# ratt-ru/tricolour

Hardware: AMD Instinct MI355X
Metric: Mvis/s flagged (bl x time x chan x corr) (higher is better)
Workload: dtype f32 data / f64 accumulators / u8 flags; 1 GPU; MeerKAT-64 slab: 252 of 2016 bl x 4 corr x 1024 time x 4096 chan per GPU (BASELINE configs[1] processed as HBM-resident baseline slabs), sum_threshold_flagger kwargs=stage1; params=stage1

## Files before the change

tricolour_amd/csrc/kernels_boxline.hpp:

```cpp
#pragma once

struct BoxDenom { float b, y; };
__device__ __forceinline__ float box_divide(float a, const BoxDenom dn, unsigned long long& okmask) {
    float q = a * dn.y;
    okmask &= __builtin_amdgcn_ballot_w64(__builtin_amdgcn_classf(q, 0x148));
    float r = __builtin_fmaf(-dn.b, q, a);
    q = __builtin_fmaf(r, dn.y, q);
    r = __builtin_fmaf(-dn.b, q, a);
    q = __builtin_fmaf(r, dn.y, q);
    return q;
}
__device__ __forceinline__ float box_divide_ieee(float a, const BoxDenom dn) { return a / dn.b; }
__device__ __forceinline__ float box_divide_checked(float a, const BoxDenom dn) {
    unsigned long long ok = ~0ull;
    const float q = box_divide(a, dn, ok);
    return ((ok >> (threadIdx.x & 63)) & 1ull) ? q : box_divide_ieee(a, dn);
}

template <int KS, typename V, typename A>
struct BoxLine {
    V R1[KS], R2[KS], R3[KS], R4[KS];
    A s1, s2, s3, s4;
    V o1, o2, o3;
    V old1, old2, old3, old4;
// ... 116 lines not shown
                const unsigned w = (unsigned)__builtin_amdgcn_raw_buffer_load_b32(frs, coff, t < n ? (int)((unsigned)(t >> 2) * rowb) : 0, 0);
                prew[q] = (t < n) ? w : 0x01010101u;
            }
        } else {
#pragma unroll
            for (int u = 0; u < PF; u++) {
                const int t = t0 + u;
                const unsigned w = (unsigned)__builtin_amdgcn_raw_buffer_load_b8(frs, c, t < n ? (int)((unsigned)t * (unsigned)C) : 0, 0);
                prew[PACKED ? 0 : u] = (t < n) ? w : 1u;
            }
        }
        if (IMG == 1) {
#pragma unroll
            for (int u = 0; u < PF; u++)
                pre[u] = __builtin_bit_cast(float, __builtin_amdgcn_raw_buffer_load_b32(drs, coff, t0 + u < n ? (int)((unsigned)(t0 + u) * rowb) : 0, 0));
        }
    };
    auto store = [&](int i, float y) {
        __builtin_amdgcn_raw_buffer_store_b32(__builtin_bit_cast(unsigned, y), ors, coff, (int)((unsigned)i * rowb), 0);
    };
    issue(0);
    for (int mb = 0; mb < total; mb += UNR) {
#pragma unroll
        for (int b = 0; b < UNR / PF; b++) {
            const int m0 = mb + b * PF;
            if (m0 < total) {
                V cur[PF];
#pragma unroll
                for (int u = 0; u < PF; u++) {
                    const bool fl = PACKED ? ((prew[u >> 2] >> (8 * (u & 3))) & 0xFFu) != 0 : prew[PACKED ? 0 : u] != 0;
                    cur[u] = (IMG == 0) ? (fl ? (V)0 : (V)1) : (fl ? (V)0 : (V)pre[u]);
                }
                issue(m0 + PF);
                const bool fast = SPLIT && m0 >= 4 * r + 3 && m0 + PF <= n;
                if (fast) {
#pragma unroll
                    for (int u = 0; u < PF; u++) {
                        V* cell = cells + (size_t)lslot * BT4;
                        if (HASL) lslot = (lslot + 1 == d) ? 0 : lslot + 1;
                        const V* ncell = cells + (size_t)lslot * BT4;
                        const float out = boxline_step<KS, V, A, HASL, true>(L, (b * PF + u) % KS, m0 + u, cur[u], n, R2x, cell, ncell, BT);
                        store(m0 + u - 3 - 4 * r, out / denom);
                        if (BOXR_SCHED_EVERY > 0 && (u % (BOXR_SCHED_EVERY > 0 ? BOXR_SCHED_EVERY : 1)) == (BOXR_SCHED_EVERY > 0 ? BOXR_SCHED_EVERY : 1) - 1) __builtin_amdgcn_sched_barrier(0);
                    }
                } else {
#pragma unroll
                    for (int u = 0; u < PF; u++) {
                        V* cell = cells + (size_t)lslot * BT4;
                        if (HASL) lslot = (lslot + 1 == d) ? 0 : lslot + 1;
                        const V* ncell = cells + (size_t)lslot * BT4;
                        const float out = boxline_step<KS, V, A, HASL, false>(L, (b * PF + u) % KS, m0 + u, cur[u], n, R2x, cell, ncell, BT);
                        const int i = m0 + u - 3 - 4 * r;
                        if (i >= 0 && i < n) store(i, out / denom);
                        if (BOXR_SCHED_EVERY > 0 && (u % (BOXR_SCHED_EVERY > 0 ? BOXR_SCHED_EVERY : 1)) == (BOXR_SCHED_EVERY > 0 ? BOXR_SCHED_EVERY : 1) - 1) __builtin_amdgcn_sched_barrier(0);
                    }
                }
            }
        }
    }
}

template <int KS, bool HASL, int IMG>
__global__ void __launch_bounds__(64, boxr_waves(KS))
k_boxt(const float* __restrict__ srcData, const uint8_t* __restrict__ srcFlags,
       float* __restrict__ dstImg, int n, int C, int r, float denom, size_t sws, size_t dws) {
    boxt_body<KS, HASL, IMG, true, boxr_pf(KS)>(srcData, srcFlags, dstImg, n, C, r, denom, sws, dws, blockIdx.y);
}

__host__ __device__ constexpr int boxt_spec_pf(int ks) { return ks <= 16 ? 64 : (ks == 32 ? 32 : 16); }
template <int KS, bool HASL>
__global__ void __launch_bounds__(64, 1)
k_boxt_spec(const float* __restrict__ srcData, const uint8_t* __restrict__ srcFlags,
            float* __restrict__ dstW, float* __restrict__ dstO, int n, int C, int r, float denom) {
    if (blockIdx.y == 0) boxt_body<KS, HASL, 0, false, boxt_spec_pf(KS)>(srcData, srcFlags, dstW, n, C, r, denom, 0, 0, 0);
    else boxt_body<KS, HASL, 1, false, boxt_spec_pf(KS)>(srcData, srcFlags, dstO, n, C, r, denom, 0, 0, 0);
}

__host__ __device__ constexpr int boxf_ts(int pf) { return pf >= 32 ? 33 : 34; }
#ifndef BOXF_DOUBLE_STAGE
#define BOXF_DOUBLE_STAGE 1
#endif
__host__ __device__ constexpr int boxf_nsub(int ks) { return (BOXF_DOUBLE_STAGE && ks <= 16 && boxr_pf_f(ks) == 16) ? 2 : 1; }
#define BOXF_TS 34
#ifndef BOXF_STREAM_AUX
#define BOXF_STREAM_AUX 0
#endif
__host__ __device__ constexpr bool boxf_panel_ok(int ks, bool hasl) { return ks <= 8 || (ks == 16 && !hasl); }
template <int KS, bool HASL, int MODE, int WPS = boxr_waves_f(KS)>
__global__ void __launch_bounds__(64, WPS)
k_boxf(const float* __restrict__ srcW, unsigned img_gap,
       float* __restrict__ dstW, float* __restrict__ dstO, const float* __restrict__ data,
       int n, int C, int ld, int r, BoxDenom denom, size_t sws_img, size_t dws, size_t ws_data,
       uint8_t* __restrict__ nanflag, float* __restrict__ dstP, size_t pws) {
    extern __shared__ float cf_ring[];
    constexpr int PF = boxr_pf_f(KS);
    static_assert(MODE != 2 || (PF / 2) % 4 == 0, "panel output: groups of four positions per lane");
    constexpr int NSUB = boxf_nsub(KS);
    constexpr int PL = PF * NSUB;
    constexpr int UNR = boxr_lcm(boxr_lcm(KS, PF), PL);
    constexpr int BT = 64;
    constexpr int LPI = 32 / PL;
    constexpr int TS = boxf_ts(PL);
    const int lane = threadIdx.x;
    const int half = lane >> 5;
    const int hl = lane & 31;
    const int c0 = blockIdx.x * 32;
    const int c = c0 + hl;
    const bool colok = c < C;
    const size_t win = blockIdx.y;
    const int R2x = 2 * r;
    const int d = R2x - KS;
    float* ring = cf_ring + lane;
    float* tiles = cf_ring + (size_t)4 * d * BT;
    float* tile = tiles + (size_t)half * PL * TS;
    if (HASL)
        for (int k = 0; k < 4 * d; k++) ring[(size_t)k * BT] = 0.0f;

    const unsigned rowb = (unsigned)C * 4u;
    const __amdgpu_buffer_rsrc_t xrs = __builtin_amdgcn_make_buffer_rsrc(
        (void*)(data + win * ws_data), 0, (int)((unsigned)n * rowb), 0x00020000);
    const __amdgpu_buffer_rsrc_t ors = __builtin_amdgcn_make_buffer_rsrc(
        (void*)(dstO + win * dws), 0, (int)((unsigned)n * rowb), 0x00020000);
    const __amdgpu_buffer_rsrc_t wrs = __builtin_amdgcn_make_buffer_rsrc(
        (void*)(dstW + win * dws), 0, (int)((unsigned)n * rowb), 0x00020000);
    const bool panel = MODE == 2 && boxf_panel_ok(KS, HASL) && dstP != nullptr;
    const __amdgpu_buffer_rsrc_t prs = __builtin_amdgcn_make_buffer_rsrc(
        (void*)(panel ? dstP + win * pws : dstW), 0, panel ? (int)((unsigned)n * rowb) : 0, 0x00020000);

    const int s_pos = hl % PL;
    const int s_line0 = hl / PL;
    const unsigned ldb = (unsigned)ld * 4u;
    const __amdgpu_buffer_rsrc_t srs = __builtin_amdgcn_make_buffer_rsrc(
        (void*)(srcW + win * sws_img), 0, (int)((img_gap + (unsigned)C * (unsigned)ld) * 4u), 0x00020000);
    const int s_off = (int)((unsigned)s_line0 * ldb) + s_pos * 4 + (half ? (int)(img_gap * 4u) : 0);
    float pre[PL];
    auto issue = [&](int t0) {
        const int sbase = (int)((unsigned)c0 * ldb) + t0 * 4;
        if (t0 + PL <= n && c0 + 32 <= C) {
#pragma unroll
            for (int j = 0; j < PL; j++)
                pre[j] = __builtin_bit_cast(float, __builtin_amdgcn_raw_buffer_load_b32(srs, s_off, sbase + (int)((unsigned)(LPI * j) * ldb), 0));
        } else {
            const bool tok = t0 + s_pos < n;
#pragma unroll
            for (int j = 0; j < PL; j++) {
                const bool ok = tok && (c0 + LPI * j + s_line0 < C);
                const float v = __builtin_bit_cast(float, __builtin_amdgcn_raw_buffer_load_b32(srs, ok ? s_off + sbase + (int)((unsigned)(LPI * j) * ldb) : 0, 0, 0));
                pre[j] = ok ? v : 0.0f;
            }
        }
    };
    auto wave_sync = [] {
        __builtin_amdgcn_fence(__ATOMIC_RELEASE, "wavefront");
        __builtin_amdgcn_wave_barrier();
        __builtin_amdgcn_fence(__ATOMIC_ACQUIRE, "wavefront");
    };
    const int hrow = (PF / 2) * half;
    const int hoff = (colok ? c : 0) * 4 + (int)((unsigned)hrow * rowb);
    const float* eb = tiles + (size_t)hrow * TS + hl;
    float dpre[PF / 2];
    auto issue_data = [&](int m0, bool fast) {
        const int i0 = m0 - 3 - 4 * r;
        if (fast) {
#pragma unroll
            for (int k = 0; k < PF / 2; k++)
                dpre[k] = __builtin_bit_cast(float, __builtin_amdgcn_raw_buffer_load_b32(xrs, hoff, (int)((unsigned)(i0 + k) * rowb), BOXF_STREAM_AUX));
        } else {
#pragma unroll
            for (int k = 0; k < PF / 2; k++) {
                const int i = i0 + hrow + k;
                const bool ok = i >= 0 && i < n;
                const float v = __builtin_bit_cast(float, __builtin_amdgcn_raw_buffer_load_b32(xrs, ok ? (colok ? c : 0) * 4 + (int)((unsigned)i * rowb) : 0, 0, 0));
                dpre[k] = ok ? v : 0.0f;
            }
        }
    };

    BoxLine<KS, float, double> L;
    L.init();
    constexpr size_t BT4 = (size_t)4 * BT;
    int lslot = 0;
    const int total = n + 4 * r + 3;
    bool line_nan = false;
    issue(0);
    for (int mb = 0; mb < total; mb += UNR) {
#pragma unroll
        for (int b = 0; b < UNR / PF; b++) {
            const int m0 = mb + b * PF;
            if (m0 < total) {
                const int ro = (b % NSUB) * PF;
                if (b % NSUB == 0) {
                    wave_sync();
#pragma unroll
                    for (int j = 0; j < PL; j++) tile[s_pos * TS + LPI * j + s_line0] = pre[j];
                    wave_sync();
                    issue(m0 + PL);
                }
                const bool fast = m0 >= 4 * r + 3 && m0 + PF <= n;
                issue_data(m0, fast);
                float xin = tile[ro * TS + hl];
                if (fast) {
#pragma unroll
                    for (int u = 0; u < PF; u++) {
                        const float xnext = (u + 1 < PF) ? tile[(ro + u + 1) * TS + hl] : 0.0f;
                        float* cell = ring + (size_t)lslot * BT4;
                        if (HASL) lslot = (lslot + 1 == d) ? 0 : lslot + 1;
                        const float* ncell = ring + (size_t)lslot * BT4;
                        tile[(ro + u) * TS + hl] = boxline_step<KS, float, double, HASL, true>(L, (b * PF + u) % KS, m0 + u, xin, n, R2x, cell, ncell, BT);
                        xin = xnext;
                        if (BOXR_SCHED_EVERY > 0 && u % (BOXR_SCHED_EVERY > 0 ? BOXR_SCHED_EVERY : 1) == 0) __builtin_amdgcn_sched_barrier(0);
                    }
                } else {
#pragma unroll
                    for (int u = 0; u < PF; u++) {
                        const float xnext = (u + 1 < PF) ? tile[(ro + u + 1) * TS + hl] : 0.0f;
                        float* cell = ring + (size_t)lslot * BT4;
                        if (HASL) lslot = (lslot + 1 == d) ? 0 : lslot + 1;
                        const float* ncell = ring + (size_t)lslot * BT4;
                        tile[(ro + u) * TS + hl] = boxline_step<KS, float, double, HASL, false>(L, (b * PF + u) % KS, m0 + u, xin, n, R2x, cell, ncell, BT);
                        xin = xnext;
                        if (BOXR_SCHED_EVERY > 0 && u % (BOXR_SCHED_EVERY > 0 ? BOXR_SCHED_EVERY : 1) == 0) __builtin_amdgcn_sched_barrier(0);
                    }
                }
                if (m0 + PF - 1 - 3 - 4 * r >= 0) {
                    wave_sync();
                    const int i0 = m0 - 3 - 4 * r;
                    unsigned long long okmask = ~0ull, active = 0;
                    float res[MODE == 2 ? PF / 2 : 1];
                    auto finish = [&](auto ieee_tag) {
                        constexpr bool IEEE = decltype(ieee_tag)::value;
#pragma unroll
                        for (int k = 0; k < PF / 2; k++) {
                            const int i = i0 + hrow + k;
                            if ((fast || (i >= 0 && i < n)) && colok) {
                                if (!IEEE) active |= __builtin_amdgcn_ballot_w64(true);
                                const float wv = IEEE ? box_divide_ieee(eb[(ro + k) * TS], denom) : box_divide(eb[(ro + k) * TS], denom, okmask);
                                const float ov = IEEE ? box_divide_ieee(eb[(PL + ro + k) * TS], denom) : box_divide(eb[(PL + ro + k) * TS], denom, okmask);
                                const float bg = (wv == 0.0f) ? NAN : ov / wv;
                                const int vo = fast ? hoff : (c * 4 + (int)((unsigned)i * rowb));
                                const int so = fast ? (int)((unsigned)(i0 + k) * rowb) : 0;
                                if (MODE == 1) {
                                    __builtin_amdgcn_raw_buffer_store_b32(__builtin_bit_cast(unsigned, fabsf(dpre[k] - bg)), ors, vo, so, BOXF_STREAM_AUX);
                                } else {
                                    __builtin_amdgcn_raw_buffer_store_b32(__builtin_bit_cast(unsigned, bg), ors, vo, so, BOXF_STREAM_AUX);
                                    res[MODE == 2 ? k : 0] = dpre[k] - bg;
                                    __builtin_amdgcn_raw_buffer_store_b32(__builtin_bit_cast(unsigned, res[MODE == 2 ? k : 0]), wrs, vo, so, BOXF_STREAM_AUX);
                                    line_nan |= isnan(bg);
                                }
                            }
                            if (BOXR_SCHED_EVERY > 0) __builtin_amdgcn_sched_barrier(0);
                        }
                    };
                    finish(std::false_type{});
                    if ((okmask & active) != active) finish(std::true_type{});
                    if (MODE == 2 && panel && colok) {
                        auto paddr = [&](int i) { return (int)((((unsigned)(i >> 6) * (unsigned)C + (unsigned)c) << 8) + ((unsigned)(i & 63) << 2)); };
#pragma unroll
                        for (int g = 0; g < PF / 8; g++) {
                            const int ig = i0 + hrow + 4 * g;
                            if (fast && (ig & 63) <= 60) {
                                typedef unsigned u4 __attribute__((ext_vector_type(4)));
                                u4 y;
#pragma unroll
                                for (int e = 0; e < 4; e++) y[e] = __builtin_bit_cast(unsigned, res[MODE == 2 ? 4 * g + e : 0]);
                                __builtin_amdgcn_raw_buffer_store_b128(y, prs, paddr(ig), 0, BOXF_STREAM_AUX);
                            } else {
#pragma unroll
                                for (int e = 0; e < 4; e++)
                                    if (fast || (ig + e >= 0 && ig + e < n))
                                        __builtin_amdgcn_raw_buffer_store_b32(__builtin_bit_cast(unsigned, res[MODE == 2 ? 4 * g + e : 0]), prs, paddr(ig + e), 0, BOXF_STREAM_AUX);
                            }
                        }
                    }
                }
            }
        }
    }
    if (MODE == 2 && line_nan && colok) nanflag[win * (size_t)C + c] = 1;
}
```

tricolour_amd/csrc/kernels_boxpipe.hpp:

```cpp
#pragma once
#include <hip/hip_runtime.h>
#include <stdint.h>
#include <type_traits>

__host__ __device__ constexpr int boxp_lc(int r, int B) { return (2 * r + 2 * B + B - 1) / B * B; }
__host__ __device__ constexpr size_t boxp_lds_bytes(int r, int B) {
    return ((size_t)4 * (boxp_lc(r, B) + B) * 64 + (size_t)2 * B * 64) * 4;
}

template <int IMG, int B, int P>
__device__ __forceinline__ void boxp_body(const float* __restrict__ srcData, const uint8_t* __restrict__ srcFlags,
                                          float* __restrict__ dst, const int n, const int C, const int r, const float denom) {
    extern __shared__ float cf_ring[];
    using V = typename std::conditional<IMG == 0, int, float>::type;
    using A = typename std::conditional<IMG == 0, int, double>::type;
    constexpr int K = B / 4;
    static_assert(K == 2 || K == 4, "block length 8 or 16");
    constexpr unsigned OOB = 0x7ffffff0u;
    const int tid = threadIdx.x, lane = tid & 63;
    const int wave = __builtin_amdgcn_readfirstlane(tid >> 6);
    const int R2 = 2 * r;
    const int Lc = boxp_lc(r, B), LcP = Lc + B;
    V* bufs = reinterpret_cast<V*>(cf_ring);
    float* outb = cf_ring + (size_t)4 * LcP * 64;
// ... 267 lines not shown
                    V* po = &fifo[wave + 1][slot * B][lane];
                    if (whole) {
#pragma unroll
                        for (int u = 0; u < B; u++) po[u * 64] = o[u];
                    } else {
#pragma unroll
                        for (int u = 0; u < B; u++) {
                            o[u] = (t0 + u >= keep_lo && t0 + u < keep_hi) ? o[u] : (V)0;
                            po[u * 64] = o[u];
                        }
                    }
                    if (slot == 0) {
#pragma unroll
                        for (int u = 0; u < B; u++) po[(NF * B + u) * 64] = o[u];
                    }
                }
                slot = slot == NF - 1 ? 0 : slot + 1;
                s0 = s0 + B >= NF * B ? s0 + B - NF * B : s0 + B;
            }
#endif
#if !(BOXQ_ABLATE & 1)
            {
                const int bs = j - 5;
                const int i0 = bs * B + PPT * wave - 4 * r;
                const float* ob = &outb[bs & 1][PPT * wave][lane];
                float a[PPT], y[PPT];
                unsigned long long okm = ~0ull;
#pragma unroll
                for (int k = 0; k < PPT; k++) { a[k] = ob[k * 64]; y[k] = box_divide(a[k], denom, okm); }
                if (okm != ~0ull) {
                    TRI_KEEP_BRANCH();
#pragma unroll
                    for (int k = 0; k < PPT; k++) y[k] = box_divide_ieee(a[k], denom);
                }
#pragma unroll
                for (int k = 0; k < PPT; k++) {
                    const int i = i0 + k;
                    const bool ok = bs >= 0 && bs < NB && i >= 0 && i < n && colok;
                    __builtin_amdgcn_raw_buffer_store_b32(__builtin_bit_cast(unsigned, y[k]), ors, (int)(ok ? (unsigned)i * rowb + coff : OOB), 0, 0);
                }
            }
#endif
            __syncthreads();
        }
    }
}

template <int KS, int IMG, int B = 16>
__global__ void __launch_bounds__(256, B == 8 ? 4 : 2)
k_boxq(const float* __restrict__ srcData, const uint8_t* __restrict__ srcFlags, float* __restrict__ dstImg,
       int n, int C, int r, BoxDenom denom, size_t sws, size_t dws) {
    boxq_body<IMG, KS, B == 8 ? boxq_prefetch8(KS / 8) : boxq_prefetch(KS), B>(srcData, srcFlags, dstImg, n, C, r, denom, sws, dws, blockIdx.y);
}
template <int KS, int IMG>
__global__ void __launch_bounds__(256, 3)
k_boxq_deep(const float* __restrict__ srcData, const uint8_t* __restrict__ srcFlags, float* __restrict__ dstImg,
            int n, int C, int r, BoxDenom denom, size_t sws, size_t dws) {
    boxq_body<IMG, KS, boxq_prefetch8(KS / 8), 8, 4>(srcData, srcFlags, dstImg, n, C, r, denom, sws, dws, blockIdx.y);
}

#ifndef BOXQF_LW
#define BOXQF_LW 64
#endif
#ifndef BOXQF_DBL
#define BOXQF_DBL 1
#endif
#ifndef BOXQF_PAIR
#define BOXQF_PAIR 1
#endif
#ifndef BOXQF_ABLATE_BARRIER
#define BOXQF_ABLATE_BARRIER 0
#endif
__host__ __device__ constexpr bool boxqf_dbl(int KS, int B) { return BOXQF_DBL && B == 8 && (KS / B) % 2 == 0; }
__host__ __device__ constexpr int boxqf_prefetch2(int nblk) { return nblk == 6 ? 3 : (nblk == 10 || nblk == 2 ? 1 : 2); }
__host__ __device__ constexpr size_t boxqf_lds_floats(int B, bool dbl) { return (size_t)(2 * ((dbl ? 5 : 4) + 3 * 4) * B * BOXQF_LW + 2 * 2 * B * BOXQF_LW); }
__host__ __device__ constexpr size_t boxqf_lds_bytes(int B, bool dbl = false) { return boxqf_lds_floats(B, dbl) * 4; }
#define BOXQF_LDS_BYTES boxqf_lds_bytes(16)
#ifndef BOXQF_P10
#define BOXQF_P10 2
#endif
__host__ __device__ constexpr int boxqf_prefetch8(int nblk) {
    return nblk == 6 ? 3 : (nblk == 8 ? 4 : (nblk == 9 ? 3 : (nblk == 10 ? BOXQF_P10 : (nblk == 12 ? 4 : nblk))));
}
#ifndef BOXQF_MINW8
#define BOXQF_MINW8 4
#endif
template <int KS, int MODE, int B = 16>
__global__ void __launch_bounds__(512, B == 8 ? BOXQF_MINW8 : 1)
k_boxqf(const float* __restrict__ srcW, unsigned img_gap, float* __restrict__ dstW, float* __restrict__ dstO,
        const float* __restrict__ data, int n, int C, int ld, int r, BoxDenom denom, size_t sws_img, size_t dws,
        size_t ws_data, uint8_t* __restrict__ nanflag) {
    constexpr int PP = B / 4;
    constexpr int FN = B / 8;
    constexpr int NBLK = KS / B;
    constexpr bool DBL = boxqf_dbl(KS, B);
    constexpr int P2 = boxqf_prefetch2(NBLK);
    constexpr int P = DBL ? 2 * P2 : (B == 8 ? boxqf_prefetch8(NBLK) : boxq_prefetch(KS));
    static_assert(KS % B == 0, "register part: whole blocks");
    static_assert(B == 8 || B == 16, "block length");
    constexpr int U = boxq_lcm(NBLK, P);
    static_assert(!DBL || U % 2 == 0, "double-block staging: an even number of iterations per trip");
    constexpr unsigned OOB = 0x7ffffff0u;
    extern __shared__ float cf_ring[];
    constexpr int LW = BOXQF_LW;
    constexpr int NF1 = DBL ? 4 : 3;
    constexpr int F1 = (NF1 + 1) * B * LW, FN3 = 4 * B * LW;
    typedef float OutT[B][LW];
    auto fifo_of = [&](int image, int stage) -> float* {
        return stage == 0 ? cf_ring + image * F1 : cf_ring + 2 * F1 + (image * 3 + stage - 1) * FN3;
    };
    OutT* outb = reinterpret_cast<OutT*>(cf_ring + 2 * F1 + 6 * FN3);
    constexpr bool PAIR = BOXQF_PAIR && B == 8 && KS <= 40;
    auto ld2 = [&](const float* fifo, int row) -> float2 {
        if (PAIR) return *reinterpret_cast<const float2*>(fifo + ((size_t)(row >> 1) * LW + (threadIdx.x & 63)) * 2);
        const float* p = fifo + (size_t)row * LW + (threadIdx.x & 63);
        return make_float2(p[0], p[LW]);
    };
    auto st2 = [&](float* fifo, int row, int line, float a, float b2) {
        if (PAIR) { *reinterpret_cast<float2*>(fifo + ((size_t)(row >> 1) * LW + line) * 2) = make_float2(a, b2); return; }
        float* p = fifo + (size_t)row * LW + line;
        p[0] = a;
        p[LW] = b2;
    };
    const int tid = threadIdx.x, lane = tid & 63;
    const int wave = __builtin_amdgcn_readfirstlane(tid >> 6);
    const int img = wave >> 2, st = wave & 3;
    const size_t win = blockIdx.y;
    const int c0 = blockIdx.x * 64;
    const int R2 = 2 * r;
    const int d = R2 - KS;
    const int NB = (n + 4 * r + B - 1) / B;
    for (int k = tid; k < 2 * F1 + 6 * FN3; k += 512) cf_ring[k] = 0.0f;

    const int s_line = (tid & 255) >> 2, s_q = tid & 3;
    const bool s_lok = c0 + s_line < C;
    const float* s_base = srcW + win * sws_img + (size_t)(img ? img_gap : 0u) + (size_t)(s_lok ? c0 + s_line : 0) * ld;
    float pre[DBL ? P2 : P][DBL ? 4 : PP];
    auto issue = [&](int blk, int q) {
        if (DBL) {
            const int p = blk * 16 + 4 * s_q;
            const float4 v = *reinterpret_cast<const float4*>(s_base + (p < n ? p : 0));
            pre[q][0] = v.x; pre[q][1] = v.y; pre[q][DBL ? 2 : 0] = v.z; pre[q][DBL ? 3 : 0] = v.w;
            return;
        }
        const int p = blk * B + PP * s_q;
        if (PP == 4) {
            const float4 v = *reinterpret_cast<const float4*>(s_base + (p < n ? p : 0));
            pre[q][0] = v.x; pre[q][1] = v.y; pre[q][PP - 2] = v.z; pre[q][PP - 1] = v.w;
        } else {
            const float2 v = *reinterpret_cast<const float2*>(s_base + (p < n ? p : 0));
            pre[q][0] = v.x; pre[q][1] = v.y;
        }
    };
    const int f_u = tid >> 6;
    const int c = c0 + lane;
    const bool colok = c < C;
    const unsigned rowb = (unsigned)C * 4u;
    const unsigned coff = (unsigned)c * 4u;
    const __amdgpu_buffer_rsrc_t xrs = __builtin_amdgcn_make_buffer_rsrc((void*)(data + win * ws_data), 0, (int)((unsigned)n * rowb), 0x00020000);
    const __amdgpu_buffer_rsrc_t ors = __builtin_amdgcn_make_buffer_rsrc((void*)(dstO + win * dws), 0, (int)((unsigned)n * rowb), 0x00020000);
    const __amdgpu_buffer_rsrc_t wrs = __builtin_amdgcn_make_buffer_rsrc((void*)(dstW + win * dws), 0, (int)((unsigned)n * rowb), 0x00020000);
    float dpre[P][FN];
    auto issue_data = [&](int blk, int q) {
#pragma unroll
        for (int h = 0; h < FN; h++) {
            const int i = blk * B + f_u + 8 * h - 4 * r;
            const bool ok = blk >= 0 && i >= 0 && i < n && colok;
            dpre[q][h] = __builtin_bit_cast(float, __builtin_amdgcn_raw_buffer_load_b32(xrs, (int)(ok ? (unsigned)i * rowb + coff : OOB), 0, 0));
        }
    };
#pragma unroll
    for (int q = 0; q < P; q++) { if (!DBL || q < P2) issue(q, q); issue_data(q - 5, q); }

    float R[KS];
#pragma unroll
    for (int k = 0; k < KS; k++) R[k] = 0.0f;
    double acc = 0.0;
    int lslot = 0;
    const int nf = st == 0 ? NF1 : 3;
    int slot = (nf * 8 - st - 1) % nf, s0 = (nf * B * 8 - (st + 1) * B - d) % (nf * B);
    int oslot = (3 * 8 - st - 1) % 3;
    float* const fin = fifo_of(img, st);
    float* const fout = fifo_of(img, st < 3 ? st + 1 : 3);
    const int keep_lo = st == 2 ? R2 : 0;
    const int keep_hi = st == 0 ? n + R2 : 0x7fffffff;
    bool line_nan = false;
    __syncthreads();

    for (int j0 = 0; j0 < NB + 5; j0 += U) {
#pragma unroll
        for (int qq = 0; qq < U; qq++) {
            const int j = j0 + qq;
            const int q = qq % P;
            const int sb = (qq % NBLK) * B;
            if (DBL) {
                if (qq % 2 == 0) {
                    const int q2 = (qq / 2) % P2;
                    const int p = j * B + 4 * s_q;
                    const bool ok = s_lok && p < n;
                    float* pf = fifo_of(img, 0);
                    const int r0 = lslot * B + 4 * s_q;
                    const float v0 = ok ? pre[q2][0] : 0.0f, v1 = ok ? pre[q2][1] : 0.0f, v2 = ok ? pre[q2][DBL ? 2 : 0] : 0.0f, v3 = ok ? pre[q2][DBL ? 3 : 0] : 0.0f;
                    st2(pf, r0, s_line, v0, v1);
                    st2(pf, r0 + 2, s_line, v2, v3);
                    if (lslot == 0 && s_q < 2) {
                        st2(pf, NF1 * B + r0, s_line, v0, v1);
                        st2(pf, NF1 * B + r0 + 2, s_line, v2, v3);
                    }
                    lslot = lslot == 0 ? 2 : 0;
                    issue(j / 2 + P2, q2);
                }
            } else {
                const int p = j * B + PP * s_q;
                const bool ok = s_lok && p < n;
                float* pf = fifo_of(img, 0);
                const int r0 = lslot * B + PP * s_q;
#pragma unroll
                for (int k = 0; k < PP; k += 2) {
                    const float va = ok ? pre[DBL ? 0 : q][k] : 0.0f, vb = ok ? pre[DBL ? 0 : q][k + 1] : 0.0f;
                    st2(pf, r0 + k, s_line, va, vb);
                    if (lslot == 0) st2(pf, 3 * B + r0 + k, s_line, va, vb);
                }
                lslot = lslot == 2 ? 0 : lslot + 1;
            }
            if (!DBL) issue(j + P, q);
            const int b = j - st - 1;
            {
                const int t0 = b * B;
                float xin[B], xdel[B], o[B];
#pragma unroll
                for (int u = 0; u < B; u += 2) {
                    const float2 a = ld2(fin, slot * B + u), d2 = ld2(fin, s0 + u);
                    xin[u] = a.x; xin[u + 1] = a.y; xdel[u] = d2.x; xdel[u + 1] = d2.y;
                }
#pragma unroll
                for (int u = 0; u < B; u++) {
                    const float old = R[sb + u];
                    R[sb + u] = xdel[u];
                    acc += (double)xin[u];
                    o[u] = (float)acc;
                    acc -= (double)old;
                }
                if (st == 3) {
                    float* ob = &outb[img * 2 + (b & 1)][0][lane];
#pragma unroll
                    for (int u = 0; u < B; u++) ob[u * LW] = o[u];
                } else {
                    const bool whole = t0 >= keep_lo && t0 + B <= keep_hi && b >= 0;
                    if (!whole) {
#pragma unroll
                        for (int u = 0; u < B; u++) o[u] = (t0 + u >= keep_lo && t0 + u < keep_hi) ? o[u] : 0.0f;
                    }
#pragma unroll
                    for (int u = 0; u < B; u += 2) st2(fout, oslot * B + u, lane, o[u], o[u + 1]);
                    if (oslot == 0) {
#pragma unroll
                        for (int u = 0; u < B; u += 2) st2(fout, 3 * B + u, lane, o[u], o[u + 1]);
                    }
                }
                slot = slot == nf - 1 ? 0 : slot + 1;
                oslot = oslot == 2 ? 0 : oslot + 1;
                s0 = s0 + B >= nf * B ? s0 + B - nf * B : s0 + B;
            }
            {
                const int bs = j - 5;
                float wq[FN], oq[FN], a0[FN], a1[FN];
                unsigned long long okm = ~0ull;
#pragma unroll
                for (int h = 0; h < FN; h++) {
                    a0[h] = outb[bs & 1][f_u + 8 * h][lane];
                    a1[h] = outb[2 + (bs & 1)][f_u + 8 * h][lane];
                    wq[h] = box_divide(a0[h], denom, okm);
                    oq[h] = box_divide(a1[h], denom, okm);
                }
                if (okm != ~0ull) {
                    TRI_KEEP_BRANCH();
#pragma unroll
                    for (int h = 0; h < FN; h++) { wq[h] = box_divide_ieee(a0[h], denom); oq[h] = box_divide_ieee(a1[h], denom); }
                }
#pragma unroll
                for (int h = 0; h < FN; h++) {
                    const int i = bs * B + f_u + 8 * h - 4 * r;
                    const bool ok = bs >= 0 && bs < NB && i >= 0 && i < n && colok;
                    const unsigned off = ok ? (unsigned)i * rowb + coff : OOB;
                    const float bg = (wq[h] == 0.0f) ? NAN : oq[h] / wq[h];
                    const float dv = dpre[q][h];
                    if (MODE == 1) {
                        __builtin_amdgcn_raw_buffer_store_b32(__builtin_bit_cast(unsigned, fabsf(dv - bg)), ors, (int)off, 0, 0);
                    } else {
                        __builtin_amdgcn_raw_buffer_store_b32(__builtin_bit_cast(unsigned, bg), ors, (int)off, 0, 0);
                        __builtin_amdgcn_raw_buffer_store_b32(__builtin_bit_cast(unsigned, dv - bg), wrs, (int)off, 0, 0);
                        line_nan |= ok && isnan(bg);
                    }
                }
            }
            issue_data(j + P - 5, q);
#if BOXQF_ABLATE_BARRIER
            asm volatile("" ::: "memory");
            __builtin_amdgcn_sched_barrier(0);
#else
            __syncthreads();
#endif
        }
    }
    if (MODE == 2 && line_nan) nanflag[win * (size_t)C + c] = 1;
}
```

tricolour_amd/csrc/kernels_elementwise.hpp:

```cpp
#pragma once

template <int VD>
__global__ void k_prepare(const void* __restrict__ vis, const uint8_t* __restrict__ iflags,
                          float* __restrict__ data, uint8_t* __restrict__ flags,
                          int T, int F, int Fa, int factor) {
    size_t idx = (size_t)blockIdx.x * blockDim.x + threadIdx.x;
    size_t NA = (size_t)T * Fa;
    if (idx >= NA) return;
    int t = (int)(idx / Fa), fo = (int)(idx % Fa);
    size_t w = blockIdx.y;
    size_t base = w * (size_t)T * F + (size_t)t * F;
    int f0 = fo * factor;
    int f1 = min(F, f0 + factor);
    float sum = 0.0f;
    int cnt = 0;
    for (int f = f0; f < f1; f++) {
        if (VD == TRI_VIS_F64) {
            const double a = fabs(reinterpret_cast<const double*>(vis)[base + f]);
            if (!iflags[base + f] && !isnan(a)) { sum = (float)((double)sum + a); cnt++; }
            continue;
        }
        float a = load_amp<VD>(vis, base + f);
        if (!iflags[base + f] && !isnan(a)) { sum += a; cnt++; }
    }
    size_t o = w * NA + idx;
    if (cnt == 0) { data[o] = 0.0f; flags[o] = 1; }
    else { data[o] = sum / (float)cnt; flags[o] = 0; }
}

__global__ void k_abs_c64(const float2* __restrict__ z, float* __restrict__ out, size_t n) {
    size_t i = (size_t)blockIdx.x * blockDim.x + threadIdx.x;
    if (i < n) out[i] = tri_hypotf(z[i].x, z[i].y);
}

template <typename T, bool PANEL = false>
__global__ void k_transpose(const T* __restrict__ src, T* __restrict__ dst, int R, int C,
                            size_t src_ws, size_t dst_ws, float denom) {
    __shared__ T tile[64][65];
    const T* s = src + (size_t)blockIdx.z * src_ws;
    T* d = dst + (size_t)blockIdx.z * dst_ws;
    int c0 = blockIdx.x * 64, r0 = blockIdx.y * 64;
    int tx = threadIdx.x, ty = threadIdx.y;
    for (int j = ty; j < 64; j += 4) {
        int r = r0 + j, c = c0 + tx;
        if (r < R && c < C) tile[j][tx] = s[(size_t)r * C + c];
    }
    __syncthreads();
    for (int j = ty; j < 64; j += 4) {
        int c = c0 + j, r = r0 + tx;
        if (r < R && c < C) {
            T v = tile[tx][j];
            if (sizeof(T) == 4 && denom != 0.0f) v = (T)((float)v / denom);
            if (PANEL) d[((size_t)blockIdx.y * C + c) * 64 + tx] = v;
            else d[(size_t)c * R + r] = v;
        }
    }
}

template <typename T>
__global__ void k_panelize(const T* __restrict__ src, T* __restrict__ dst, int L, int C, size_t ws) {
    const size_t i = (size_t)blockIdx.x * blockDim.x + threadIdx.x;
    if (i >= (size_t)L * C) return;
    const int l = (int)(i / C), c = (int)(i % C);
    dst[blockIdx.y * ws + ((size_t)(c >> 6) * L + l) * 64 + (c & 63)] = src[blockIdx.y * ws + i];
}
template <typename T>
__global__ void k_unpanel_w(const T* __restrict__ src, T* __restrict__ dst, int L, int C, size_t ws) {
    const size_t i = (size_t)blockIdx.x * blockDim.x + threadIdx.x;
    if (i >= (size_t)L * C) return;
    const int l = (int)(i / C), c = (int)(i % C);
    dst[blockIdx.y * ws + i] = src[blockIdx.y * ws + ((size_t)(c >> 6) * L + l) * 64 + (c & 63)];
}
template <typename T>
__global__ void k_unpanel(const T* __restrict__ src, T* __restrict__ dst, int L, int C) {
    const size_t i = (size_t)blockIdx.x * blockDim.x + threadIdx.x;
    if (i >= (size_t)L * C) return;
    const int l = (int)(i / C), c = (int)(i % C);
    dst[i] = src[((size_t)(c >> 6) * L + l) * 64 + (c & 63)];
}

template <bool COPY, bool ZERO>
__global__ __launch_bounds__(256) void k_transpose_u8w(const uint8_t* __restrict__ src, uint8_t* __restrict__ dst,
                                                       uint8_t* __restrict__ copy, float* __restrict__ data, int R, int C,
                                                       size_t src_ws, size_t dst_ws, size_t copy_ws, size_t data_ws) {
    __shared__ unsigned tile[128][17];
    const uint8_t* s = src + (size_t)blockIdx.z * src_ws;
    uint8_t* d = dst + (size_t)blockIdx.z * dst_ws;
    const int c0 = blockIdx.x * 64, r0 = blockIdx.y * 128;
    const int tid = threadIdx.x;
    {
        const int tx = tid & 15, ty = tid >> 4;
        const int c = c0 + 4 * tx;
#pragma unroll
        for (int j = 0; j < 8; j++) {
            const int rr = ty + 16 * j, r = r0 + rr;
            unsigned v = 0;
            if (r < R && c < C) {
                v = *reinterpret_cast<const unsigned*>(s + (size_t)r * C + c);
                if (COPY) *reinterpret_cast<unsigned*>(copy + (size_t)blockIdx.z * copy_ws + (size_t)r * C + c) = v;
            }
            tile[rr][tx] = v;
        }
    }
    __syncthreads();
    const int bx = tid & 31, q0 = tid >> 5;
    const int r = r0 + 4 * bx;
    if (r >= R) return;
#pragma unroll
    for (int h = 0; h < 2; h++) {
        const int q = q0 + 8 * h;
        const unsigned a0 = tile[4 * bx][q], a1 = tile[4 * bx + 1][q], a2 = tile[4 * bx + 2][q], a3 = tile[4 * bx + 3][q];
        const unsigned t0 = __builtin_amdgcn_perm(a1, a0, 0x05010400u), t1 = __builtin_amdgcn_perm(a1, a0, 0x07030602u);
        const unsigned u0 = __builtin_amdgcn_perm(a3, a2, 0x05010400u), u1 = __builtin_amdgcn_perm(a3, a2, 0x07030602u);
        const unsigned o[4] = {__builtin_amdgcn_perm(u0, t0, 0x05040100u), __builtin_amdgcn_perm(u0, t0, 0x07060302u),
                               __builtin_amdgcn_perm(u1, t1, 0x05040100u), __builtin_amdgcn_perm(u1, t1, 0x07060302u)};
#pragma unroll
        for (int b = 0; b < 4; b++) {
            const int c = c0 + 4 * q + b;
            if (c >= C) break;
            *reinterpret_cast<unsigned*>(d + (size_t)c * R + r) = o[b];
            if (ZERO && o[b]) {
                const unsigned f = o[b];
                float4* pd = reinterpret_cast<float4*>(data + (size_t)blockIdx.z * data_ws + (size_t)c * R + r);
                float4 x = *pd;
                const bool dirty = ((f & 0xFFu) && __float_as_uint(x.x)) || ((f & 0xFF00u) && __float_as_uint(x.y)) ||
                                   ((f & 0xFF0000u) && __float_as_uint(x.z)) || ((f & 0xFF000000u) && __float_as_uint(x.w));
                if (dirty)
                    *pd = make_float4((f & 0xFFu) ? 0.0f : x.x, (f & 0xFF00u) ? 0.0f : x.y, (f & 0xFF0000u) ? 0.0f : x.z,
                                      (f & 0xFF000000u) ? 0.0f : x.w);
            }
        }
    }
}

__global__ void k_build_wo(const float* __restrict__ data, const uint8_t* __restrict__ flags,
                           float* __restrict__ w, float* __restrict__ o, size_t nper,
                           size_t sws, size_t dws) {
    size_t i = (size_t)blockIdx.x * blockDim.x + threadIdx.x;
    if (i >= nper) return;
    size_t win = blockIdx.y;
    bool fl = flags[win * sws + i] != 0;
    w[win * dws + i] = fl ? 0.0f : 1.0f;
    o[win * dws + i] = fl ? 0.0f : data[win * sws + i];
}

__global__ void k_build_wo4(const float* __restrict__ data, const uint8_t* __restrict__ flags,
                            float* __restrict__ w, float* __restrict__ o, size_t n4per,
                            size_t sws, size_t dws) {
    size_t i = (size_t)blockIdx.x * blockDim.x + threadIdx.x;
    if (i >= n4per) return;
    size_t win = blockIdx.y;
    uchar4 f = reinterpret_cast<const uchar4*>(flags + win * sws)[i];
    float4 d = reinterpret_cast<const float4*>(data + win * sws)[i];
    reinterpret_cast<float4*>(w + win * dws)[i] =
        make_float4(f.x ? 0.0f : 1.0f, f.y ? 0.0f : 1.0f, f.z ? 0.0f : 1.0f, f.w ? 0.0f : 1.0f);
    reinterpret_cast<float4*>(o + win * dws)[i] =
        make_float4(f.x ? 0.0f : d.x, f.y ? 0.0f : d.y, f.z ? 0.0f : d.z, f.w ? 0.0f : d.w);
}

template <int MODE>
__global__ void k_masked_div(const float* __restrict__ w, float* __restrict__ o,
                             const float* __restrict__ data, size_t nper, size_t ws_wo,
                             size_t ws_data, float denom, uint8_t* __restrict__ nanflag, int C) {
    size_t i = (size_t)blockIdx.x * blockDim.x + threadIdx.x;
    if (i >= nper) return;
    size_t win = blockIdx.y;
    float wv = w[win * ws_wo + i];
    float ov = o[win * ws_wo + i];
    if (denom != 0.0f) { wv = wv / denom; ov = ov / denom; }
    float bg = (wv == 0.0f) ? NAN : ov / wv;
    if (MODE != 1 && nanflag && isnan(bg)) nanflag[win * (size_t)C + (i % C)] = 1;
    if (MODE == 1) bg = fabsf(data[win * ws_data + i] - bg);
    o[win * ws_wo + i] = bg;
    if (MODE == 2) const_cast<float*>(w)[win * ws_wo + i] = data[win * ws_data + i] - bg;
}

template <bool TWOD>
__global__ void k_reject(const float* __restrict__ resid, uint8_t* __restrict__ flags,
                         const double* __restrict__ med, const int* __restrict__ chunk_of,
                         double scale, int L, int C, int G, size_t ws_resid, size_t ws_flags) {
    size_t i = (size_t)blockIdx.x * blockDim.x + threadIdx.x;
    if (i >= (size_t)L * C) return;
    size_t win = blockIdx.y;
    int l = (int)(i / C), c = (int)(i % C);
    int g = chunk_of[l];
    double m = TWOD ? med[win * G + g] : med[(size_t)c * G + g];
    double thr = m * scale;
    if ((double)resid[win * ws_resid + i] > thr) flags[win * ws_flags + i] = 1;
}

__global__ void k_colinterp(float* __restrict__ a, int L, int C, size_t ws,
                            const uint8_t* __restrict__ nanflag, const float* __restrict__ data,
                            size_t ws_data, float* __restrict__ resid, float* __restrict__ panel, size_t ws_panel) {
    int c = blockIdx.x * blockDim.x + threadIdx.x;
    if (c >= C) return;
    if (nanflag && !nanflag[(size_t)blockIdx.y * C + c]) return;
    float* x = a + (size_t)blockIdx.y * ws + c;
    const size_t Cs = (size_t)C;
    int last = -1;
    float lastv = 0.0f;
    int run = 0;
    constexpr int PFI = 64;
    for (int i0 = 0; i0 < L; i0 += PFI) {
// ... 237 lines not shown
    size_t i = (size_t)blockIdx.x * blockDim.x + threadIdx.x;
    if (i >= n4) return;
    uchar4 f = reinterpret_cast<const uchar4*>(iflags)[i];
    float a[4];
    if (VD == TRI_VIS_C64) {
        float4 z0 = reinterpret_cast<const float4*>(vis)[2 * i];
        float4 z1 = reinterpret_cast<const float4*>(vis)[2 * i + 1];
        a[0] = tri_hypotf(z0.x, z0.y); a[1] = tri_hypotf(z0.z, z0.w);
        a[2] = tri_hypotf(z1.x, z1.y); a[3] = tri_hypotf(z1.z, z1.w);
    } else {
        float4 z = reinterpret_cast<const float4*>(vis)[i];
        a[0] = fabsf(z.x); a[1] = fabsf(z.y); a[2] = fabsf(z.z); a[3] = fabsf(z.w);
    }
    unsigned char fl[4] = {f.x, f.y, f.z, f.w};
    float o[4];
    unsigned char of[4];
#pragma unroll
    for (int k = 0; k < 4; k++) {
        bool bad = fl[k] != 0 || isnan(a[k]);
        o[k] = bad ? 0.0f : (0.0f + a[k]) / 1.0f;
        of[k] = bad ? 1 : 0;
    }
    reinterpret_cast<float4*>(data)[i] = make_float4(o[0], o[1], o[2], o[3]);
    reinterpret_cast<uchar4*>(flags)[i] = make_uchar4(of[0], of[1], of[2], of[3]);
}

template <int VD>
__global__ void k_amplitude4(const void* __restrict__ vis, float* __restrict__ ampl,
                             uint8_t* __restrict__ iter, uint16_t* __restrict__ nanmask, size_t n4) {
    size_t i = (size_t)blockIdx.x * blockDim.x + threadIdx.x;
    if (i >= n4) return;
    float a[4];
    bool vn[4];
    if (VD == TRI_VIS_C64) {
        float4 z0 = reinterpret_cast<const float4*>(vis)[2 * i];
        float4 z1 = reinterpret_cast<const float4*>(vis)[2 * i + 1];
        a[0] = tri_hypotf(z0.x, z0.y); a[1] = tri_hypotf(z0.z, z0.w);
        a[2] = tri_hypotf(z1.x, z1.y); a[3] = tri_hypotf(z1.z, z1.w);
        vn[0] = isnan(z0.x) || isnan(z0.y); vn[1] = isnan(z0.z) || isnan(z0.w);
        vn[2] = isnan(z1.x) || isnan(z1.y); vn[3] = isnan(z1.z) || isnan(z1.w);
    } else {
        float4 z = reinterpret_cast<const float4*>(vis)[i];
        a[0] = fabsf(z.x); a[1] = fabsf(z.y); a[2] = fabsf(z.z); a[3] = fabsf(z.w);
        vn[0] = isnan(z.x); vn[1] = isnan(z.y); vn[2] = isnan(z.z); vn[3] = isnan(z.w);
    }
#pragma unroll
    for (int k = 0; k < 4; k++) a[k] = (0.0f + a[k]) / 1.0f;
    reinterpret_cast<float4*>(ampl)[i] = make_float4(a[0], a[1], a[2], a[3]);
    const unsigned nanb = (isnan(a[0]) ? 1u : 0u) | (isnan(a[1]) ? 0x100u : 0u) | (isnan(a[2]) ? 0x10000u : 0u) |
                          (isnan(a[3]) ? 0x1000000u : 0u);
    if (nanb) reinterpret_cast<unsigned*>(iter)[i] |= nanb;
    unsigned m = ((vn[0] ? 1u : 0u) | (vn[1] ? 2u : 0u) | (vn[2] ? 4u : 0u) | (vn[3] ? 8u : 0u)) << (4 * (threadIdx.x & 3));
    m |= __shfl_xor(m, 1, 64);
    m |= __shfl_xor(m, 2, 64);
    if ((threadIdx.x & 3) == 0) nanmask[i >> 2] = (uint16_t)m;
}

__global__ void k_zero_flagged4(const uint8_t* __restrict__ flags, float* __restrict__ data, size_t n4per,
                                size_t ws_flags, size_t ws_data) {
    size_t i = (size_t)blockIdx.x * blockDim.x + threadIdx.x;
    if (i >= n4per) return;
    size_t win = blockIdx.y;
    const unsigned f = reinterpret_cast<const unsigned*>(flags + win * ws_flags)[i];
    if (f == 0) return;
    float4* pd = reinterpret_cast<float4*>(data + win * ws_data) + i;
    float4 d = *pd;
    *pd = make_float4((f & 0xFFu) ? 0.0f : d.x, (f & 0xFF00u) ? 0.0f : d.y, (f & 0xFF0000u) ? 0.0f : d.z,
                      (f & 0xFF000000u) ? 0.0f : d.w);
}

template <int OP>
__global__ void k_u8_op16(const uint8_t* __restrict__ a, uint8_t* __restrict__ b, size_t n16per,
                          size_t ws_a, size_t ws_b) {
    size_t i = (size_t)blockIdx.x * blockDim.x + threadIdx.x;
    if (i >= n16per) return;
    size_t win = blockIdx.y;
    uint4 va = reinterpret_cast<const uint4*>(a + win * ws_a)[i];
    uint4* pb = reinterpret_cast<uint4*>(b + win * ws_b) + i;
    if (OP == 0) *pb = va;
    else if (OP == 1) *pb = or4(*pb, va);
    else *pb = make_uint4(nz_bytes(va.x), nz_bytes(va.y), nz_bytes(va.z), nz_bytes(va.w));
}

__global__ void k_spec_rows(const uint8_t* __restrict__ spec, uint8_t* __restrict__ rows, int Fa, int Wn) {
    size_t i = (size_t)blockIdx.x * blockDim.x + threadIdx.x;
    if (i >= (size_t)Fa * Wn) return;
    int w = (int)(i / Fa), f = (int)(i % Fa);
    rows[i] = spec[(size_t)f * Wn + w];
}

__global__ void k_or_spec16(uint8_t* __restrict__ flags, const uint8_t* __restrict__ spec_rows, int T, int Fa16) {
    size_t i = (size_t)blockIdx.x * blockDim.x + threadIdx.x;
    if (i >= (size_t)T * Fa16) return;
    size_t win = blockIdx.y;
    int f16 = (int)(i % Fa16);
    uint4 sp = reinterpret_cast<const uint4*>(spec_rows + win * (size_t)Fa16 * 16)[f16];
    uint4* pf = reinterpret_cast<uint4*>(flags + win * (size_t)T * Fa16 * 16) + i;
    *pf = or4(*pf, sp);
}

__global__ void k_or_spec_more16(uint8_t* __restrict__ flags, const uint8_t* __restrict__ spec_rows,
                                 const uint8_t* __restrict__ more, int T, int Fa16) {
    size_t i = (size_t)blockIdx.x * blockDim.x + threadIdx.x;
    if (i >= (size_t)T * Fa16) return;
    size_t win = blockIdx.y;
    int f16 = (int)(i % Fa16);
    uint4 sp = reinterpret_cast<const uint4*>(spec_rows + win * (size_t)Fa16 * 16)[f16];
    size_t a = win * (size_t)T * Fa16 + i;
    uint4* pf = reinterpret_cast<uint4*>(flags) + a;
    *pf = or4(or4(*pf, sp), reinterpret_cast<const uint4*>(more)[a]);
}

__global__ void k_or_spec_ft16(uint8_t* __restrict__ flagsFT, const uint8_t* __restrict__ spec_rows, int T16, int Fa) {
    size_t i = (size_t)blockIdx.x * blockDim.x + threadIdx.x;
    if (i >= (size_t)T16 * Fa) return;
    size_t win = blockIdx.y;
    int f = (int)(i / T16);
    if (!spec_rows[win * (size_t)Fa + f]) return;
    reinterpret_cast<uint4*>(flagsFT + win * (size_t)T16 * 16 * Fa)[i] = make_uint4(0x01010101u, 0x01010101u, 0x01010101u, 0x01010101u);
}

__global__ void k_combine16(const uint8_t* __restrict__ spec_rows, const uint8_t* __restrict__ tflags,
                            const uint8_t* __restrict__ fflags, uint8_t* __restrict__ comb, int T,
                            int Fa16, int lo, int hi) {
    size_t i = (size_t)blockIdx.x * blockDim.x + threadIdx.x;
    if (i >= (size_t)T * Fa16) return;
    size_t win = blockIdx.y;
    int t = (int)(i / Fa16), f16 = (int)(i % Fa16);
    size_t base = win * (size_t)T * Fa16;
    int t0 = max(t + lo, 0), t1 = min(t + hi, T);
    uint4 v = make_uint4(0, 0, 0, 0);
    if (t1 > t0) {
        v = reinterpret_cast<const uint4*>(spec_rows + win * (size_t)Fa16 * 16)[f16];
        const uint4* tp = reinterpret_cast<const uint4*>(tflags) + base;
        const uint4* fp = reinterpret_cast<const uint4*>(fflags) + base;
        for (int tt = t0; tt < t1; tt++) {
            size_t a = (size_t)tt * Fa16 + f16;
            v = or4(v, or4(tp[a], fp[a]));
        }
    }
    reinterpret_cast<uint4*>(comb)[base + i] = v;
}

template <bool TPANEL>
__global__ __launch_bounds__(64) void k_combine_dilate16(const uint8_t* __restrict__ spec_rows, const uint8_t* __restrict__ tflags,
                                                        const uint8_t* __restrict__ fflags, uint8_t* __restrict__ dil,
                                                        int* __restrict__ rowcnt, int T, int F16, int lo, int hi) {
    const int lane = threadIdx.x;
    const int f16 = blockIdx.x * 64 + lane;
    const int t = blockIdx.y;
    const size_t win = blockIdx.z;
    const size_t base = win * (size_t)T * F16;
    const int t0 = max(t + lo, 0), t1 = min(t + hi, T);
    const bool in = f16 < F16;
    uint4 c = make_uint4(0, 0, 0, 0);
    if (in && t1 > t0) {
        c = reinterpret_cast<const uint4*>(spec_rows + win * (size_t)F16 * 16)[f16];
        const uint4* tp = reinterpret_cast<const uint4*>(tflags) + base;
        const uint4* fp = reinterpret_cast<const uint4*>(fflags) + base;
        for (int tt = t0; tt < t1; tt++) {
            size_t a = (size_t)tt * F16 + f16;
            size_t at = TPANEL ? ((size_t)(f16 >> 2) * T + tt) * 4 + (f16 & 3) : a;
            c = or4(c, or4(tp[at], fp[a]));
        }
    }
    auto edge = [&](int g, int b) -> unsigned {
        if (g < 0 || g >= F16 || t1 <= t0) return 0u;
        unsigned v = spec_rows[(win * (size_t)F16 + g) * 16 + b];
        for (int tt = t0; tt < t1; tt++) {
            size_t a = (base + (size_t)tt * F16 + g) * 16 + b;
            size_t at = TPANEL ? (base + ((size_t)(g >> 2) * T + tt) * 4 + (g & 3)) * 16 + b : a;
// ... 646 lines not shown
```

tricolour_amd/csrc/kernels_reject_tile.hpp:

```cpp
#pragma once

#ifndef MRT_CWIN
#define MRT_CWIN 4u
#endif
#ifndef MRT_DWIN
#define MRT_DWIN 2u
#endif
#ifndef MRT_WCAND
#define MRT_WCAND 384
#endif
#ifndef MRT_WUND
#define MRT_WUND 192
#endif
#define MRT_PARW 16
#define MRT_ANY_ROUND2 0x10000u
struct MrtPar {
    unsigned lo, S, wlo, whi;
    double thrA, thrB;
    unsigned ncand, nund, below1, status;
    unsigned pad[2];
    double thrP;
};
static_assert(sizeof(MrtPar) == MRT_PARW * 4, "parameter record");

// ... 57 lines not shown
    if (hi < lo) { give_up(); return; }
    if (hi > (16u << 23) && lo < hi - (16u << 23)) lo = hi - (16u << 23);
    int S = 0;
    {
        const unsigned span = hi - lo;
        while (S < 31 && (span >> S) >= 2046u) S++;
    }
#pragma unroll
    for (int u = 0; u < SEL_BINS / 256; u++) hist[u * 256 + tid] = 0;
    __syncthreads();
#pragma unroll
    for (int rr = 0; rr < 64; rr++) {
        const unsigned k = keys[rr];
        if (k != 0xFFFFFFFFu) {
            const unsigned b = k < lo ? 0u : min(((k - lo) >> S) + 1u, 2047u);
            atomicAdd(&hist[b], 1u);
        }
    }
    __syncthreads();
    unsigned v[8];
    {
        uint4 q0 = reinterpret_cast<const uint4*>(hist)[2 * tid];
        uint4 q1 = reinterpret_cast<const uint4*>(hist)[2 * tid + 1];
        v[0] = q0.x; v[1] = q0.y; v[2] = q0.z; v[3] = q0.w;
        v[4] = q1.x; v[5] = q1.y; v[6] = q1.z; v[7] = q1.w;
    }
    unsigned sacc = 0;
#pragma unroll
    for (int j = 0; j < 8; j++) sacc += v[j];
    unsigned inc = sacc;
#pragma unroll
    for (int o = 1; o < 64; o <<= 1) {
        unsigned t2 = __shfl_up(inc, o, 64);
        if (lane >= o) inc += t2;
    }
    if (lane == 63) sh[wave] = inc;
    __syncthreads();
    unsigned woff = 0, ns = 0;
#pragma unroll
    for (int w2 = 0; w2 < 4; w2++) {
        unsigned t2 = sh[w2];
        if (w2 < wave) woff += t2;
        ns += t2;
    }
    const unsigned kk = ns >> 1, exc = woff + inc - sacc;
    if (ns > 0 && kk >= exc && kk < exc + sacc) {
        unsigned c = exc;
        int j = 0;
#pragma unroll
        for (int q = 0; q < 7; q++)
            if (j == q && kk >= c + v[q]) { c += v[q]; j = q + 1; }
        sh_bin = 8u * tid + j;
    }
    __syncthreads();
    if (ns < 4096) { give_up(); return; }
    if (tid == 0) {
        const unsigned bp = sh_bin;
        MrtPar p{};
        p.lo = lo; p.S = (unsigned)S;
        const unsigned cw = S >= 17 ? max(MRT_CWIN >> (S - 17), 2u) : min(MRT_CWIN << (17 - S), 200u);
        const unsigned dw = S >= 17 ? max(MRT_DWIN >> (S - 17), 1u) : min(MRT_DWIN << (17 - S), 100u);
        p.wlo = bp > cw + 1u ? bp - cw : 1u;
        p.whi = bp + cw < 2046u ? bp + cw : 2046u;
        const unsigned dlo = bp > dw + 1u ? bp - dw : 1u;
        const unsigned dhi = bp + dw < 2046u ? bp + dw : 2046u;
        const unsigned long long kB64 = (unsigned long long)lo + ((unsigned long long)dhi << S) - 1ull;
        const unsigned kA = lo + ((dlo - 1u) << S), kB = kB64 > 0x7F7FFFFFull ? 0x7F7FFFFFu : (unsigned)kB64;
        p.thrA = (double)__uint_as_float(kA) * scale;
        p.thrB = (double)__uint_as_float(kB) * scale;
        const unsigned long long kP64 = (unsigned long long)lo + ((unsigned long long)(bp > 0u ? bp - 1u : 0u) << S) + ((1ull << S) >> 1);
        const unsigned kP = min(max((unsigned)min(kP64, 0x7F7FFFFFull), kA), kB);
        p.thrP = (double)__uint_as_float(kP) * scale;
        p.status = 1;
        *par = p;
    }
}

#ifndef MRT_PASS_WAVES
#define MRT_PASS_WAVES 4
#endif
__global__ void __launch_bounds__(256, MRT_PASS_WAVES)
k_mr_pass(const float* __restrict__ resid, const uint8_t* __restrict__ flags_in, uint8_t* __restrict__ flags_out,
          uint8_t* __restrict__ flags_t4, const int64_t* __restrict__ chunk_ends, int L, int C4, int G,
          size_t ws_resid, size_t ws_flags, unsigned* __restrict__ gscratch, size_t scratch_ws, size_t ccap, size_t ucap, unsigned round) {
    __shared__ unsigned hist[SEL_BINS + 64];
    __shared__ unsigned tile[64][65];
    __shared__ unsigned lcand[4][MRT_WCAND];
    __shared__ uint2 lund[4][MRT_WUND];
    const size_t win = blockIdx.z;
    const int tid = threadIdx.x, lane = tid & 63, wave = __builtin_amdgcn_readfirstlane(tid >> 6);
    const int tx = lane, ty = wave;
    if (round == 2 && !(reinterpret_cast<const MrtPar*>(gscratch + win * scratch_ws)->pad[0] & MRT_ANY_ROUND2)) return;
    int g = 0, l0 = 0, c1 = 0;
    {
        int y = blockIdx.y;
        for (g = 0; g < G; g++) {
            const int a = (int)chunk_ends[g], b = (int)chunk_ends[g + 1];
            const int nt = (b - a + 63) / 64;
            if (y < nt) { l0 = a + 64 * y; c1 = b; break; }
            y -= nt;
        }
        if (g >= G) return;
    }
    const MrtLayout lay{gscratch + win * scratch_ws, G, ccap, ucap};
    MrtPar* par = lay.par(g);
    __shared__ unsigned sh_status;
    if (tid == 0) sh_status = __hip_atomic_load(&par->status, __ATOMIC_RELAXED, __HIP_MEMORY_SCOPE_AGENT);
    __syncthreads();
    if (sh_status != round) return;
    const unsigned lo = par->lo, S = par->S, wlo = par->wlo, wspan = par->whi - par->wlo;
    const double thrA = par->thrA, thrB = par->thrB, thrP = par->thrP;
    const int w0 = blockIdx.x * 64, w = w0 + tx;
    const float4* r4 = reinterpret_cast<const float4*>(resid + win * ws_resid);
    const unsigned* fin = reinterpret_cast<const unsigned*>(flags_in + win * ws_flags);
    unsigned* fout = reinterpret_cast<unsigned*>(flags_out + win * ws_flags);
    unsigned* ft = reinterpret_cast<unsigned*>(flags_t4 + win * ws_flags);
    constexpr unsigned OOBR = 0x7ffffff0u;
    const __amdgpu_buffer_rsrc_t fors = __builtin_amdgcn_make_buffer_rsrc((void*)fout, 0, (int)((unsigned)L * (unsigned)C4 * 4u), 0x00020000);
#pragma unroll
    for (int u = 0; u < SEL_BINS / 256; u++) hist[u * 256 + tid] = 0;
    float4 rv[16];
    unsigned f[16];
#pragma unroll
    for (int q = 0; q < 16; q++) {
        const int l = l0 + ty + 4 * q;
        const size_t i = (l < c1 && w < C4) ? (size_t)l * C4 + w : (size_t)l0 * C4;
        rv[q] = r4[i];
        f[q] = fin[i];
    }
    __syncthreads();
    unsigned mb1 = 0;
    unsigned ccnt = 0, ucnt = 0;
#pragma unroll
    for (int q = 0; q < 16; q++) {
        const int l = l0 + ty + 4 * q;
        const bool valid = l < c1 && w < C4;
        const unsigned i = (unsigned)l * (unsigned)C4 + (unsigned)w;
        const float xv[4] = {rv[q].x, rv[q].y, rv[q].z, rv[q].w};
        unsigned fn = f[q];
#pragma unroll
        for (int k4 = 0; k4 < 4; k4++) {
            const unsigned k = __float_as_uint(xv[k4]) & 0x7FFFFFFFu;
            const bool unfl = valid && ((f[q] >> (8 * k4)) & 0xFFu) == 0u;
            const unsigned b = k < lo ? 0u : min(((k - lo) >> S) + 1u, 2047u);
            atomicAdd(&hist[unfl ? b : SEL_BINS + (unsigned)lane], 1u);
            mb1 = max(mb1, (unfl && b < wlo) ? k + 1u : 0u);
            const bool inwin = unfl && (b - wlo <= wspan);
            const unsigned long long cm = __builtin_amdgcn_ballot_w64(inwin);
            if (cm) {
                const unsigned pos = ccnt + __builtin_amdgcn_mbcnt_hi((unsigned)(cm >> 32), __builtin_amdgcn_mbcnt_lo((unsigned)cm, 0u));
                if (inwin && pos < MRT_WCAND) lcand[wave][pos] = k;
                ccnt += (unsigned)__builtin_popcountll(cm);
                if (ccnt > MRT_WCAND) {
                    const bool sp = inwin && pos >= MRT_WCAND;
                    const unsigned long long sm = __builtin_amdgcn_ballot_w64(sp);
                    unsigned b2 = 0;
                    if (lane == 0 && sm) b2 = atomicAdd(&par->ncand, (unsigned)__builtin_popcountll(sm));
                    b2 = (unsigned)__builtin_amdgcn_readfirstlane((int)b2);
                    const size_t at = (size_t)b2 + __builtin_amdgcn_mbcnt_hi((unsigned)(sm >> 32), __builtin_amdgcn_mbcnt_lo((unsigned)sm, 0u));
                    if (sp && at < ccap) lay.cand(g)[at] = k;
                }
            }
            const double dx = (double)xv[k4];
            const bool gtB = dx > thrB, gtA = dx > thrA, gtP = dx > thrP;
            fn |= gtP ? (1u << (8 * k4)) : 0u;
            const bool und = unfl && gtA && !gtB;
            const unsigned long long um = __builtin_amdgcn_ballot_w64(und);
            if (um) {
                const unsigned pos = ucnt + __builtin_amdgcn_mbcnt_hi((unsigned)(um >> 32), __builtin_amdgcn_mbcnt_lo((unsigned)um, 0u));
                const uint2 ent = make_uint2(i * 4u + (unsigned)k4, __float_as_uint(xv[k4]));
                if (und && pos < MRT_WUND) lund[wave][pos] = ent;
                ucnt += (unsigned)__builtin_popcountll(um);
                if (ucnt > MRT_WUND) {
                    const bool sp = und && pos >= MRT_WUND;
                    const unsigned long long sm = __builtin_amdgcn_ballot_w64(sp);
                    unsigned b2 = 0;
                    if (lane == 0 && sm) b2 = atomicAdd(&par->nund, (unsigned)__builtin_popcountll(sm));
                    b2 = (unsigned)__builtin_amdgcn_readfirstlane((int)b2);
                    const size_t at = (size_t)b2 + __builtin_amdgcn_mbcnt_hi((unsigned)(sm >> 32), __builtin_amdgcn_mbcnt_lo((unsigned)sm, 0u));
                    if (sp && at < ucap) reinterpret_cast<uint2*>(lay.und(g))[at] = ent;
                }
            }
        }
        __builtin_amdgcn_raw_buffer_store_b32(fn, fors, (int)(valid ? i * 4u : OOBR), 0, 0);
        tile[ty + 4 * q][tx] = fn;
    }
    ccnt = min(ccnt, (unsigned)MRT_WCAND);
    ucnt = min(ucnt, (unsigned)MRT_WUND);
    mb1 = wave_max_u32(mb1);
    unsigned cbase = 0, ubase = 0;
    if (lane == 0) {
        if (mb1) atomicMax(&par->below1, mb1);
        if (ccnt) cbase = atomicAdd(&par->ncand, ccnt);
        if (ucnt) ubase = atomicAdd(&par->nund, ucnt);
    }
    cbase = (unsigned)__builtin_amdgcn_readfirstlane((int)cbase);
    ubase = (unsigned)__builtin_amdgcn_readfirstlane((int)ubase);
    __syncthreads();
    for (int j = ty; j < 64; j += 4) {
        const int wq = w0 + j, l = l0 + tx;
        if (l < c1 && wq < C4) ft[(size_t)wq * L + l] = tile[tx][j];
    }
    if (round == 1) {
        unsigned* ghist = lay.hist(g);
#pragma unroll
        for (int u = 0; u < SEL_BINS / 256; u++) {
            const unsigned h = hist[u * 256 + tid];
            if (h) atomicAdd(&ghist[u * 256 + tid], h);
        }
    }
    unsigned* gc = lay.cand(g);
// ... 145 lines not shown
```

tricolour_amd/csrc/tricolour_amd.hip:

```cpp
#include <unordered_set>
#include "tri_common.hpp"
#include "kernels_elementwise.hpp"
#include "kernels_median.hpp"
#include "kernels_reject.hpp"
#include "kernels_reject_tile.hpp"
#include "kernels_boxfilter.hpp"
#include "kernels_boxline.hpp"
#include "kernels_boxpipe.hpp"
#include "kernels_boxweight.hpp"
#include "kernels_boxexact.hpp"
#include "kernels_sumthreshold.hpp"
#include "kernels_scan.hpp"
#include "kernels_sir.hpp"
#include "kernels_linerms.hpp"
#include "steps/kernels_blint.hpp"
#include "steps/ldev/kernels_ldev.hpp"
#include "steps/ins/kernels_ins.hpp"
#include "steps/hyst/kernels_hyst.hpp"
#include "steps/quality/kernels_quality.hpp"
#include "steps/hist/kernels_hist.hpp"
#include "steps/medz/kernels_medz.hpp"

namespace {

// ... 58 lines not shown

struct Plan {
    int64_t T, F, Fa, avg, G;
    int64_t r0max, r1max;
    int64_t PT, PF;
    int nit;
    bool vec;
    int64_t maxchunk;
    StWin swT, swF;
};

int make_stwin(const int64_t* w, int64_t nw, double rho, StWin* s) {
    memset(s, 0, sizeof(*s));
    if (nw <= 0) return set_err(TRI_EINVAL, "no SumThreshold window fits the data (np.max of an empty window list)");
    if (nw > TRI_MAX_WINDOWS) return set_err(TRI_EINVAL, "too many windows");
    s->nw = (int)nw;
    int off = 0, d = 0, maxw = 0;
    for (int j = 0; j < nw; j++) {
        if (w[j] <= 0) return set_err(TRI_EINVAL, "SumThreshold window of size %lld (the reference fails here with a broadcasting ValueError)", (long long)w[j]);
        s->w[j] = (int)w[j];
        s->tf[j] = std::pow(rho, std::log2((double)w[j]));
        s->scale[j] = (double)(float)(1.0 / (double)w[j]);
        s->ringoff[j] = off;
        off += (int)w[j];
        s->delay[j] = d;
        d += (int)w[j] - 1;
        maxw = std::max(maxw, (int)w[j]);
    }
    s->delay[nw] = d;
    s->ringtot = off;
    s->acccap = d + 1;
    s->maxw = maxw;
    return TRI_OK;
}

int make_plan(int64_t T, int64_t F, const tri_params* p, Plan* pl) {
    if (T <= 0 || F <= 0) return set_err(TRI_EINVAL, "empty window (ntime=%lld, nchan=%lld)", (long long)T, (long long)F);
    if (p->average_freq < 1 || p->average_freq > 255) return set_err(TRI_EUNSUPPORTED, "average_freq must be in [1, 255]");
    if (p->n_chunk_ends < 2 || !p->chunk_ends) return set_err(TRI_EINVAL, "freq_chunks must be >= 1");
    if (p->background_iterations < 0 || p->num_major_iterations < 0) return set_err(TRI_EINVAL, "negative iteration count");
    pl->T = T; pl->F = F; pl->avg = p->average_freq;
    pl->Fa = (F + pl->avg - 1) / pl->avg;
    pl->G = p->n_chunk_ends - 1;
    for (int64_t g = 0; g < p->n_chunk_ends; g++) {
        if (p->chunk_ends[g] < 0 || p->chunk_ends[g] > pl->Fa || (g > 0 && p->chunk_ends[g] < p->chunk_ends[g - 1]))
            return set_err(TRI_EINVAL, "freq chunk ends must be non-decreasing within [0, averaged channels]");
    }
    if (p->chunk_ends[0] != 0 || p->chunk_ends[pl->G] != pl->Fa) return set_err(TRI_EINVAL, "freq chunk ends must start at 0 and end at the averaged channel count");
    pl->nit = (int)p->background_iterations;
    pl->maxchunk = 0;
    for (int64_t g = 0; g + 1 < p->n_chunk_ends; g++) pl->maxchunk = std::max(pl->maxchunk, p->chunk_ends[g + 1] - p->chunk_ends[g]);
    pl->vec = (pl->avg == 1 && F % 16 == 0 && T % 4 == 0);
    int64_t emax = std::max<int64_t>(pl->nit, 1);
    pl->r0max = box_radius((double)emax * p->spike_width_time);
    pl->r1max = box_radius((double)emax * p->spike_width_freq);
    if (pl->r0max > (1 << 20) || pl->r1max > (1 << 20)) return set_err(TRI_EUNSUPPORTED, "spike width too large");
    pl->PT = T + 4 * pl->r0max;
    pl->PF = pl->Fa + 4 * pl->r1max;
    int rc = TRI_OK;
    memset(&pl->swT, 0, sizeof(pl->swT));
    memset(&pl->swF, 0, sizeof(pl->swF));
    if (p->num_major_iterations > 0) {
        rc = make_stwin(p->windows_time, p->n_windows_time, p->rho, &pl->swT);
        if (rc) return rc;
        rc = make_stwin(p->windows_freq, p->n_windows_freq, p->rho, &pl->swF);
        if (rc) return rc;
    }
    if (T * pl->Fa >= ((int64_t)1 << 31) || T * F >= ((int64_t)1 << 31))
        return set_err(TRI_EUNSUPPORTED, "a single window must hold fewer than 2^31 samples");
    return TRI_OK;
}

#define TRI_MAX_CHUNKS 255
struct ChunkTab {
    int n;
    int64_t ends[TRI_MAX_CHUNKS + 1];
};

struct Ws {
    float *dataTF, *dataFT, *Aw, *Ao, *Bw, *Bo;
    uint8_t *iter, *flagsTF, *flagsFT, *bgfTF, *bgfFT, *tflTF, *fflFT, *fflTF, *comb, *dil;
    float* residP;
    int *rowcnt, *colcnt;
    double* med;
    float *sdata, *sw, *so, *sres;
    uint8_t *sflags, *sbgf, *sout, *srows;
    uint16_t* nanmask;
    int* itab;
    float* srowsf;
    uint8_t* srowsu;
    double* smed;
    double* ring;
    uint8_t* acc;
    int64_t* d_chunk_ends;
    int64_t* d_tends;
    int64_t *segC_start, *segC_len;
    int64_t *segB_start, *segB_len;
    int64_t *segT_start, *segT_len;
    int* d_chunk_of;
    size_t total;
};

static void carve(const Plan& pl, int64_t Wb, void* base, size_t cap, bool dry, Ws* ws) {
    Bump b(base, cap, dry);
    size_t W = (size_t)Wb, T = (size_t)pl.T, F = (size_t)pl.F, Fa = (size_t)pl.Fa, G = (size_t)pl.G;
    size_t N = T * Fa;
    ws->d_chunk_ends = b.get<int64_t>(G + 1);
    ws->d_tends = b.get<int64_t>(2);
    ws->segC_start = b.get<int64_t>(G);
    ws->segC_len = b.get<int64_t>(G);
    ws->segB_start = b.get<int64_t>(G);
    ws->segB_len = b.get<int64_t>(G);
    ws->segT_start = b.get<int64_t>(1);
    ws->segT_len = b.get<int64_t>(1);
    ws->d_chunk_of = b.get<int>(Fa);
    ws->iter = b.get<uint8_t>(W * T * F);
    ws->dataTF = b.get<float>(W * N);
    ws->dataFT = b.get<float>(W * N);
    ws->Aw = b.get<float>(W * 2 * (size_t)pl.PT * Fa);
    ws->Ao = dry ? nullptr : ws->Aw + (size_t)pl.PT * Fa;
    ws->Bw = b.get<float>(W * (size_t)pl.PF * T);
    ws->Bo = b.get<float>(W * (size_t)pl.PF * T);
    ws->flagsTF = b.get<uint8_t>(W * N);
    ws->flagsFT = b.get<uint8_t>(W * N);
    ws->tflTF = b.get<uint8_t>(W * N);
    ws->fflFT = b.get<uint8_t>(W * N);
    ws->fflTF = b.get<uint8_t>(W * N);
    ws->bgfTF = b.get<uint8_t>(W * N);
    ws->bgfFT = b.get<uint8_t>(W * N);
    ws->comb = b.get<uint8_t>(W * N);
    ws->dil = b.get<uint8_t>(W * T * F);
    ws->residP = dry ? nullptr : reinterpret_cast<float*>(ws->bgfTF);
    ws->rowcnt = b.get<int>(W * T);
    ws->colcnt = b.get<int>(W * F);
    ws->nanmask = b.get<uint16_t>(W * N / 16 + 8);
    ws->itab = b.get<int>(3 * W * (size_t)cdiv(Fa, INTERP_SEG) * std::max<size_t>(T, 1));
    ws->med = b.get<double>(W * std::max(Fa, T * G));
    size_t PS = (size_t)pl.PF;
    ws->sdata = b.get<float>(Fa * W);
    ws->sw = b.get<float>(PS * W);
    ws->so = b.get<float>(PS * W);
    ws->sres = b.get<float>(Fa * W);
    ws->sflags = b.get<uint8_t>(Fa * W);
    ws->sbgf = b.get<uint8_t>(Fa * W);
    ws->sout = b.get<uint8_t>(Fa * W);
    ws->srows = b.get<uint8_t>(Fa * W);
    ws->srowsf = b.get<float>(Fa * W);
    ws->srowsu = b.get<uint8_t>(Fa * W);
    ws->smed = b.get<double>(W * G);
    size_t thrT = W * Fa, thrF = W * T * G;
    size_t ringn = std::max(thrT * (size_t)pl.swT.ringtot, thrF * (size_t)pl.swF.ringtot);
    size_t accn = std::max(thrT * (size_t)pl.swT.acccap, thrF * (size_t)pl.swF.acccap);
    ws->ring = b.get<double>(ringn);
    ws->acc = b.get<uint8_t>(accn);
    ws->total = b.off;
}

static inline dim3 grid1(size_t n, size_t W) { return dim3((unsigned)cdiv((int64_t)n, 256), (unsigned)W, 1); }

}

__global__ void k_tables(ChunkTab ct, int T, int Fa, int64_t* chunk_ends, int64_t* tends,
                         int64_t* segC_start, int64_t* segC_len, int64_t* segB_start,
                         int64_t* segB_len, int64_t* segT_start, int64_t* segT_len,
                         int* chunk_of) {
    int i = blockIdx.x * blockDim.x + threadIdx.x;
    int G = ct.n - 1;
    if (i <= G) chunk_ends[i] = ct.ends[i];
    if (i < G) {
        segC_start[i] = ct.ends[i];
        segC_len[i] = ct.ends[i + 1] - ct.ends[i];
        segB_start[i] = ct.ends[i] * T;
        segB_len[i] = (ct.ends[i + 1] - ct.ends[i]) * T;
    }
    if (i == 0) { tends[0] = 0; tends[1] = T; segT_start[0] = 0; segT_len[0] = T; }
    if (i < Fa) {
        int g = 0;
        while (g < G - 1 && !(i >= ct.ends[g] && i < ct.ends[g + 1])) g++;
        chunk_of[i] = g;
    }
}

__global__ void k_gather_col_f32(const float* __restrict__ a, float* __restrict__ out, int L, int C, int col) {
    int i = blockIdx.x * blockDim.x + threadIdx.x;
    if (i < L) out[i] = a[(size_t)i * C + col];
}
__global__ void k_gather_col_u8(const uint8_t* __restrict__ a, uint8_t* __restrict__ out, int L, int C, int col) {
    int i = blockIdx.x * blockDim.x + threadIdx.x;
    if (i < L) out[i] = a[(size_t)i * C + col];
}
__global__ void k_normalise_flags(const uint8_t* __restrict__ a, uint8_t* __restrict__ b, size_t n) {
    size_t i = (size_t)blockIdx.x * blockDim.x + threadIdx.x;
    if (i < n) b[i] = a[i] ? 1 : 0;
}

extern "C" size_t tri_workspace_bytes(int64_t batch_windows, int64_t ntime, int64_t nchan,
                                      const tri_params* p) {
    Plan pl;
    if (!p || batch_windows <= 0 || make_plan(ntime, nchan, p, &pl) != TRI_OK) return 0;
    Ws ws;
    carve(pl, batch_windows, nullptr, 0, true, &ws);
    return ws.total;
}

extern "C" int tri_prepare_params(int64_t ntime, int64_t nchan, double outlier_nsigma,
                                  const double* windows_time, int64_t n_windows_time,
                                  const double* windows_freq, int64_t n_windows_freq,
                                  double background_reject, int64_t background_iterations,
                                  double spike_width_time, double spike_width_freq,
                                  int64_t time_extend, int64_t freq_extend, int64_t freq_chunks,
                                  int64_t average_freq, double flag_all_time_frac,
                                  double flag_all_freq_frac, double rho,
                                  int64_t num_major_iterations, int64_t* chunk_ends_buf,
                                  int64_t chunk_cap, tri_params* out) {
    if (!out || !chunk_ends_buf) return set_err(TRI_EINVAL, "NULL output");
    if (ntime <= 0 || nchan <= 0) return set_err(TRI_EINVAL, "empty window");
    if (average_freq < 1) return set_err(TRI_EINVAL, "average_freq must be >= 1");
// ... 480 lines not shown
            break;
        }
    }
    LAUNCHCHK();
    return TRI_OK;
}

bool st_use_pipe(const StWin& sw) {
    static const bool off = is1(getenv("TRI_ST_NO_PIPE"));
    return !off && sw.nw >= 1 && sw.nw <= 8 && stp_lds_bytes(sw) <= 160 * 1024;
}

enum class StKernel { Dyn, Fused, Mask, MaskPanel, Pipe };

int st_launch(hipStream_t st, StKernel k, const StWin& sw, const float* data, const double* med, uint8_t* out,
              const int64_t* d_chunk_ends, double thr_scale, int L, int C, int G, size_t ws_data, size_t ws_out, int64_t W,
              double* ring, uint8_t* acc) {
    int blk = C >= 256 ? 256 : (C >= 128 ? 128 : 64);
    if (const char* e = getenv("TRI_ST_BLK")) { int b = atoi(e); if (b >= 64 && b <= ST_MAXBLK && C >= b) blk = b; }
    const dim3 grid((unsigned)cdiv(C, blk), (unsigned)G, (unsigned)W);
    StFusedArgs fa;
    for (int j = 0; j < 4; j++) fa.tf[j] = sw.tf[j < sw.nw ? j : 0];
    if (k == StKernel::MaskPanel)
        hipLaunchKernelGGL((k_colst_mask<1, 2, 4, 8, true>), grid, dim3(blk), 0, st, data, med, out, d_chunk_ends, fa, thr_scale, L, C, G, ws_data, ws_out);
    else if (k == StKernel::Mask)
        hipLaunchKernelGGL((k_colst_mask<1, 2, 4, 8>), grid, dim3(blk), 0, st, data, med, out, d_chunk_ends, fa, thr_scale, L, C, G, ws_data, ws_out);
    else if (k == StKernel::Fused)
        hipLaunchKernelGGL((k_colst_fused<1, 2, 4, 8>), grid, dim3(blk), 0, st, data, med, out, d_chunk_ends, fa, thr_scale, L, C, G, ws_data, ws_out);
    else if (k == StKernel::Pipe) {
        HIPCHK(lds_optin_all(160 * 1024, &k_colst_pipe));
        hipLaunchKernelGGL(k_colst_pipe, dim3((unsigned)cdiv(C, 64), (unsigned)G, (unsigned)W), dim3(64 * sw.nw), stp_lds_bytes(sw), st,
                           data, med, out, d_chunk_ends, sw, stp_plan(sw), thr_scale, L, C, G, ws_data, ws_out);
    } else
        hipLaunchKernelGGL(k_colst_dyn, grid, dim3(blk), 0, st, data, med, out, ring, acc, d_chunk_ends, sw, thr_scale, L, C, G, ws_data, ws_out);
    LAUNCHCHK();
    return TRI_OK;
}

int launch_colst(const Run& r, const StWin& sw, const float* data, const double* med,
                 uint8_t* out, const int64_t* d_chunk_ends, int L, int C, int G, size_t ws_data,
                 size_t ws_out, int64_t W, bool panel = false) {
    StKernel k;
    if (st_use_fused(sw)) {
        if (panel && !(st_use_mask(L, C) && C % 64 == 0)) return set_err(TRI_EUNSUPPORTED, "panel images: lane-mask SumThreshold kernel on 64-column panels only");
        k = panel ? StKernel::MaskPanel : (st_use_mask(L, C) ? StKernel::Mask : StKernel::Fused);
    } else if (panel) {
        return set_err(TRI_EUNSUPPORTED, "panel images: windows (1, 2, 4, 8) only");
    } else {
        k = st_use_pipe(sw) ? StKernel::Pipe : StKernel::Dyn;
    }
    const double thr_scale = r.p->outlier_nsigma * TRI_MAD_NORMAL;
    return st_launch(r.st, k, sw, data, med, out, d_chunk_ends, thr_scale, L, C, G, ws_data, ws_out, W, r.ws.ring, r.ws.acc);
}

int launch_interp(const Run& r, float* a, int L, int C, size_t ws, int64_t W, const uint8_t* nanflag,
                  const float* data, size_t ws_data, float* resid, float* panel = nullptr, size_t ws_panel = 0) {
    static const bool one_pass = is1(getenv("TRI_INTERP_ONE_PASS"));
    const int nseg = (int)cdiv(L, INTERP_SEG);
    if (one_pass || nseg < 2 || nseg > 65535) {
        hipLaunchKernelGGL(k_colinterp, dim3((unsigned)cdiv(C, 256), (unsigned)W), dim3(256), 0, r.st, a, L, C, ws, nanflag, data, ws_data, resid, panel, ws_panel);
    } else {
        dim3 grid((unsigned)cdiv(C, 64), (unsigned)nseg, (unsigned)W);
        hipLaunchKernelGGL(k_interp_scan, grid, dim3(64), 0, r.st, (const float*)a, L, C, ws, nanflag, r.ws.itab);
        hipLaunchKernelGGL(k_interp_fix, grid, dim3(64), 0, r.st, a, L, C, ws, (const int*)r.ws.itab, data, ws_data, resid, panel, ws_panel);
    }
    LAUNCHCHK();
    return TRI_OK;
}

template <typename T>
int launch_transpose(const Run& r, const T* src, T* dst, int R, int C, size_t sws, size_t dws,
                     int64_t W, float denom = 0.0f, bool panel = false) {
    dim3 grid((unsigned)cdiv(C, 64), (unsigned)cdiv(R, 64), (unsigned)W);
    if (panel) {
        if (R % 64 != 0) return set_err(TRI_EUNSUPPORTED, "panel output needs a multiple of 64 columns");
        hipLaunchKernelGGL((k_transpose<T, true>), grid, dim3(64, 4), 0, r.st, src, dst, R, C, sws, dws, denom);
        LAUNCHCHK();
        return TRI_OK;
    }
    if (sizeof(T) == 1 && R % 4 == 0 && C % 4 == 0 && sws % 4 == 0 && dws % 4 == 0 &&
        ((uintptr_t)src % 4 == 0) && ((uintptr_t)dst % 4 == 0)) {
        dim3 gridw((unsigned)cdiv(C, 64), (unsigned)cdiv(R, 128), (unsigned)W);
        hipLaunchKernelGGL((k_transpose_u8w<false, false>), gridw, dim3(256), 0, r.st, (const uint8_t*)src, (uint8_t*)dst,
                           (uint8_t*)nullptr, (float*)nullptr, R, C, sws, dws, (size_t)0, (size_t)0);
        LAUNCHCHK();
        return TRI_OK;
    }
    hipLaunchKernelGGL(k_transpose<T>, grid, dim3(64, 4), 0, r.st, src, dst, R, C, sws, dws, denom);
    LAUNCHCHK();
    return TRI_OK;
}


template <int OP>
int launch_u8(const Run& r, const uint8_t* a, uint8_t* b, size_t nper, size_t ws_a, size_t ws_b, int64_t W) {
    if (r.pl.vec && nper % 16 == 0 && ws_a % 16 == 0 && ws_b % 16 == 0) {
        hipLaunchKernelGGL(k_u8_op16<OP>, grid1(nper / 16, W), dim3(256), 0, r.st, a, b, nper / 16, ws_a, ws_b);
    } else if (OP == 0) {
        for (int64_t w = 0; w < W; w++)
            hipLaunchKernelGGL(k_copy_u8, dim3((unsigned)cdiv(nper, 256)), dim3(256), 0, r.st, a + w * ws_a, b + w * ws_b, nper);
    } else if (OP == 1) {
        hipLaunchKernelGGL(k_or, grid1(nper, W), dim3(256), 0, r.st, b, a, nper, ws_b, ws_a);
    } else {
        for (int64_t w = 0; w < W; w++)
            hipLaunchKernelGGL(k_normalise_flags, dim3((unsigned)cdiv(nper, 256)), dim3(256), 0, r.st, a + w * ws_a, b + w * ws_b, nper);
    }
    LAUNCHCHK();
    return TRI_OK;
}

template <int MODE>
int launch_masked_div(const Run& r, const float* w, float* o, const float* data, size_t nper, size_t ws_wo, size_t ws_data, int64_t W, float denom = 0.0f,
                      uint8_t* nanflag = nullptr, int C = 1) {
    if (nper % 4 == 0 && ws_wo % 4 == 0 && ws_data % 4 == 0 && (nanflag == nullptr || C % 4 == 0) && ((uintptr_t)w % 16 == 0) && ((uintptr_t)o % 16 == 0))
        hipLaunchKernelGGL(k_masked_div4<MODE>, grid1(nper / 4, W), dim3(256), 0, r.st, w, o, data, nper / 4, ws_wo, ws_data, denom, nanflag, C);
    else
        hipLaunchKernelGGL(k_masked_div<MODE>, grid1(nper, W), dim3(256), 0, r.st, w, o, data, nper, ws_wo, ws_data, denom, nanflag, C);
    LAUNCHCHK();
    return TRI_OK;
}

int launch_sub(const Run& r, const float* a, const float* b, float* out, size_t nper, size_t ws_a, size_t ws_b, size_t ws_o, int64_t W) {
    if (nper % 4 == 0 && ws_a % 4 == 0 && ws_b % 4 == 0 && ws_o % 4 == 0 && ((uintptr_t)a % 16 == 0) && ((uintptr_t)b % 16 == 0) && ((uintptr_t)out % 16 == 0))
        hipLaunchKernelGGL(k_sub4, grid1(nper / 4, W), dim3(256), 0, r.st, a, b, out, nper / 4, ws_a, ws_b, ws_o);
    else
        hipLaunchKernelGGL(k_sub, grid1(nper, W), dim3(256), 0, r.st, a, b, out, nper, ws_a, ws_b, ws_o);
    LAUNCHCHK();
    return TRI_OK;
}

static bool filter_no_tin() { static const bool v = is1(getenv("TRI_FILTER_NO_TIN")); return v; }
bool colfilter_t_usable(int rad) { return !filter_no_tin() && rad > 0 && rad <= 16; }

int launch_colfilter_t(const Run& r, const float* srcW, const float* srcO, float* dstW, float* dstO,
                       int n, int C, int ld, int rad, size_t sws_img, size_t dws, int64_t W, float* deferred_denom) {
    float denom = box_denominator(rad);
    size_t lds = ((size_t)4 * 2 * rad * CFT_BT + (size_t)CFT_PF * (CFT_BT + 1)) * sizeof(float);
    HIPCHK(lds_optin_all(160 * 1024, &k_colfilter_lds_t<false>, &k_colfilter_lds_t<true>));
    dim3 grid((unsigned)cdiv(C, CFT_BT), (unsigned)W, 2);
    if (deferred_denom) *deferred_denom = denom;
    const auto k = deferred_denom ? &k_colfilter_lds_t<false> : &k_colfilter_lds_t<true>;
    hipLaunchKernelGGL(k, grid, dim3(CFT_BT), lds, r.st, srcW, srcO, dstW, dstO, n, C, ld, rad, denom, sws_img, dws);
    LAUNCHCHK();
    return TRI_OK;
}

bool colfilter_tf_usable(int rad) {
    static const bool off = is1(getenv("TRI_FILTER_NO_FUSED_DIV"));
    return !off && colfilter_t_usable(rad);
}

template <int MODE>
int launch_colfilter_tf(const Run& r, const float* srcW, const float* srcO, float* dstW, float* dstO, const float* data,
                        int n, int C, int ld, int rad, size_t sws_img, size_t dws, size_t ws_data, int64_t W, uint8_t* nanflag) {
    float denom = box_denominator(rad);
    size_t lds = (size_t)2 * ((size_t)4 * 2 * rad * CFF_BT + (size_t)CFT_PF * (CFF_BT + 1)) * sizeof(float);
    HIPCHK(lds_optin_all(160 * 1024, &k_colfilter_lds_tf<MODE>));
    dim3 grid((unsigned)cdiv(C, CFF_BT), (unsigned)W);
    hipLaunchKernelGGL(k_colfilter_lds_tf<MODE>, grid, dim3(2 * CFF_BT), lds, r.st, srcW, srcO, dstW, dstO, data, n, C, ld, rad,
                       denom, sws_img, dws, ws_data, nanflag);
    LAUNCHCHK();
    return TRI_OK;
}

template <int KS, int MODE>
int launch_boxf_ks(const Run& r, const float* srcW, const float* srcO, float* dstW, float* dstO, const float* data,
                   int n, int C, int ld, int rad, size_t sws_img, size_t dws, size_t ws_data, int64_t W, uint8_t* nanflag,
                   float* dstP, size_t pws, bool* wroteP) {
    const BoxDenom denom = box_reciprocal(box_denominator(rad));
    const int d = 2 * rad - KS;
    if (!(MODE == 2 && boxf_panel_ok(KS, d > 0))) dstP = nullptr;
    if (dstP && wroteP) *wroteP = true;
    const size_t lds = ((size_t)4 * d * 64 + (size_t)2 * boxr_pf_f(KS) * boxf_nsub(KS) * boxf_ts(boxr_pf_f(KS) * boxf_nsub(KS))) * sizeof(float);
    if (srcO <= srcW || ((uint64_t)(srcO - srcW) + (uint64_t)C * ld) * 4u >= (1ull << 31))
        return set_err(TRI_EUNSUPPORTED, "fused frequency stage: the data image must follow the weight image within 2^31 bytes");
    const unsigned gap = (unsigned)(srcO - srcW);
    HIPCHK(lds_optin_all(160 * 1024, &k_boxf<KS, true, MODE>));
    dim3 grid((unsigned)cdiv(C, 32), (unsigned)W);
    auto k = d > 0 ? &k_boxf<KS, true, MODE> : &k_boxf<KS, false, MODE>;
    if constexpr (KS == 32) {
        if (d > 14) { k = &k_boxf<KS, true, MODE, 1>; HIPCHK(lds_optin_all(160 * 1024, k)); }
    }
    hipLaunchKernelGGL(k, grid, dim3(64), lds, r.st, srcW, gap, dstW, dstO, data, n, C, ld, rad, denom, sws_img, dws, ws_data, nanflag, dstP, pws);
    LAUNCHCHK();
    return TRI_OK;
}

#ifndef BOXQF_MIN_2R
#define BOXQF_MIN_2R 34
#endif
#ifndef BOXQF_FEW_WAVES
#define BOXQF_FEW_WAVES 2048
#endif
#ifndef BOXQF_B8_DEFAULT
#define BOXQF_B8_DEFAULT 1
#endif
#ifndef BOXQF_B8_MAX2R
#define BOXQF_B8_MAX2R 88
#endif
template <int KS, int MODE, int B = 16>
int launch_boxqf_ks(const Run& r, const float* srcW, unsigned gap, float* dstW, float* dstO, const float* data,
                    int n, int C, int ld, int rad, size_t sws_img, size_t dws, size_t ws_data, int64_t W, uint8_t* nanflag) {
    HIPCHK(lds_optin_all(160 * 1024, &k_boxqf<KS, MODE, B>));
    const BoxDenom denom = box_reciprocal(box_denominator(rad));
    dim3 grid((unsigned)cdiv(C, 64), (unsigned)W);
    hipLaunchKernelGGL((k_boxqf<KS, MODE, B>), grid, dim3(512), boxqf_lds_bytes(B, boxqf_dbl(KS, B)), r.st, srcW, gap, dstW, dstO, data, n, C, ld, rad,
                       denom, sws_img, dws, ws_data, nanflag);
    LAUNCHCHK();
    return TRI_OK;
}

template <int MODE>
int launch_boxf(const Run& r, int ks, const float* srcW, const float* srcO, float* dstW, float* dstO, const float* data,
                int n, int C, int ld, int rad, size_t sws_img, size_t dws, size_t ws_data, int64_t W, uint8_t* nanflag,
                float* dstP = nullptr, size_t pws = 0, bool* wroteP = nullptr) {
    if (MODE != 2 || n % 64 != 0) dstP = nullptr;
    {
        static const bool off = is1(getenv("TRI_FILTER_NO_PIPE_F"));
        const int kq = boxq_pick_ks(rad);
        const bool few = (int64_t)W * cdiv(C, 32) < BOXQF_FEW_WAVES;
        const bool want = g_boxq_override == 1 || (g_boxq_override < 0 && !off && (2 * rad >= BOXQF_MIN_2R || (few && 2 * rad >= 16)));
        if (want && kq > 0 && srcO > srcW && n % 4 == 0 && ld % 4 == 0 && sws_img % 4 == 0 && (uint64_t)(srcO - srcW) % 4 == 0 &&
            ((uintptr_t)srcW % 16 == 0) && ((uint64_t)(srcO - srcW) + (uint64_t)C * ld) * 4u < (1ull << 31) &&
            (uint64_t)n * (uint64_t)C * 4u < (1ull << 31)) {
            const unsigned gap = (unsigned)(srcO - srcW);
            static const int b8 = [] { const char* e = getenv("TRI_FILTER_PIPE_F_B8"); return e ? atoi(e) : BOXQF_B8_DEFAULT; }();
            if (b8 && g_boxq_b8_override != 0 && 2 * rad >= 16 && 2 * rad < BOXQF_B8_MAX2R) {
                switch (2 * rad / 8 * 8) {
                    case 16: return launch_boxqf_ks<16, MODE, 8>(r, srcW, gap, dstW, dstO, data, n, C, ld, rad, sws_img, dws, ws_data, W, nanflag);
                    case 24: return launch_boxqf_ks<24, MODE, 8>(r, srcW, gap, dstW, dstO, data, n, C, ld, rad, sws_img, dws, ws_data, W, nanflag);
                    case 32: return launch_boxqf_ks<32, MODE, 8>(r, srcW, gap, dstW, dstO, data, n, C, ld, rad, sws_img, dws, ws_data, W, nanflag);
                    case 40: return launch_boxqf_ks<40, MODE, 8>(r, srcW, gap, dstW, dstO, data, n, C, ld, rad, sws_img, dws, ws_data, W, nanflag);
                    case 48: return launch_boxqf_ks<48, MODE, 8>(r, srcW, gap, dstW, dstO, data, n, C, ld, rad, sws_img, dws, ws_data, W, nanflag);
#if BOXQF_B8_MAX2R > 56
                    case 56: return launch_boxqf_ks<56, MODE, 8>(r, srcW, gap, dstW, dstO, data, n, C, ld, rad, sws_img, dws, ws_data, W, nanflag);
                    case 64: return launch_boxqf_ks<64, MODE, 8>(r, srcW, gap, dstW, dstO, data, n, C, ld, rad, sws_img, dws, ws_data, W, nanflag);
#endif
#if BOXQF_B8_MAX2R > 72
                    case 72: return launch_boxqf_ks<72, MODE, 8>(r, srcW, gap, dstW, dstO, data, n, C, ld, rad, sws_img, dws, ws_data, W, nanflag);
                    case 80:
                        if (MODE == 1) return launch_boxqf_ks<80, 1, 8>(r, srcW, gap, dstW, dstO, data, n, C, ld, rad, sws_img, dws, ws_data, W, nanflag);
                        break;
#endif
#if BOXQF_B8_MAX2R > 88
                    case 96: return launch_boxqf_ks<96, MODE, 8>(r, srcW, gap, dstW, dstO, data, n, C, ld, rad, sws_img, dws, ws_data, W, nanflag);
#endif
                }
            }
            switch (kq) {
                case 16: return launch_boxqf_ks<16, MODE>(r, srcW, gap, dstW, dstO, data, n, C, ld, rad, sws_img, dws, ws_data, W, nanflag);
                case 32: return launch_boxqf_ks<32, MODE>(r, srcW, gap, dstW, dstO, data, n, C, ld, rad, sws_img, dws, ws_data, W, nanflag);
                case 48: return launch_boxqf_ks<48, MODE>(r, srcW, gap, dstW, dstO, data, n, C, ld, rad, sws_img, dws, ws_data, W, nanflag);
                case 64: return launch_boxqf_ks<64, MODE>(r, srcW, gap, dstW, dstO, data, n, C, ld, rad, sws_img, dws, ws_data, W, nanflag);
                case 80: return launch_boxqf_ks<80, MODE>(r, srcW, gap, dstW, dstO, data, n, C, ld, rad, sws_img, dws, ws_data, W, nanflag);
                case 96: return launch_boxqf_ks<96, MODE>(r, srcW, gap, dstW, dstO, data, n, C, ld, rad, sws_img, dws, ws_data, W, nanflag);
            }
        }
    }
    switch (ks) {
        case 8: return launch_boxf_ks<8, MODE>(r, srcW, srcO, dstW, dstO, data, n, C, ld, rad, sws_img, dws, ws_data, W, nanflag, dstP, pws, wroteP);
        case 16: return launch_boxf_ks<16, MODE>(r, srcW, srcO, dstW, dstO, data, n, C, ld, rad, sws_img, dws, ws_data, W, nanflag, dstP, pws, wroteP);
        case 32: return launch_boxf_ks<32, MODE>(r, srcW, srcO, dstW, dstO, data, n, C, ld, rad, sws_img, dws, ws_data, W, nanflag, dstP, pws, wroteP);
        case 64: return launch_boxf_ks<64, MODE>(r, srcW, srcO, dstW, dstO, data, n, C, ld, rad, sws_img, dws, ws_data, W, nanflag, dstP, pws, wroteP);
        case 80: return launch_boxf_ks<80, MODE>(r, srcW, srcO, dstW, dstO, data, n, C, ld, rad, sws_img, dws, ws_data, W, nanflag, dstP, pws, wroteP);
    }
    return set_err(TRI_EINVAL, "no register-ring kernel for %d slots", ks);
}

thread_local int g_boxx_override = -1;
thread_local unsigned long long g_boxx_last_stats[2] = {0, 0};
#ifndef BOXX_MIN_R
#define BOXX_MIN_R 56
#endif
int boxx_pick_l(int rad, int n) {
    static const bool env_off = is1(getenv("TRI_FILTER_NO_EXACT"));
    static const int force_nti = [] { const char* e = getenv("TRI_BOXX_NTI"); return e ? atoi(e) : 0; }();
    if (g_boxx_override == 0 || (g_boxx_override < 0 && (env_off || rad < BOXX_MIN_R))) return 0;
    if (rad < 1 || n % 4 != 0) return 0;
    const int64_t P = (int64_t)n + 4 * (int64_t)rad;
    struct Cand { int nti, l; };
    static const Cand cands[] = {{128, 37}, {128, 41}, {256, 17}, {256, 19}, {256, 21}, {256, 25}};
    for (const Cand& c : cands) {
        if (force_nti && c.nti != force_nti) continue;
        if (c.nti == 128 && (P <= 128 * 17 || rad < 64)) continue;
        if ((int64_t)c.nti * c.l < P || c.l > 2 * rad + 1 || (2 * rad + 1) / c.l > BOXX_AMAX) continue;
        if (boxx_lds_bytes(c.nti, c.l, rad) > 159 * 1024) continue;
        return c.l | (c.nti << 8);
    }
    return 0;
}
static bool boxx_recip_ok(int rad) { return rad <= 128 || rad == 166 || rad == 221 || rad == 277 || rad == 397 || rad == 795; }

template <int NTI, int L, int MODE>
int launch_boxx_l(const Run& r, const float* srcW, unsigned gap, const float* data, const uint8_t* mask, float* outA, float* outB,
                  int n, int C, int ld, int rad, size_t sws_img, size_t ws_data, size_t ws_mask, size_t ws_outA, size_t ws_outB,
                  int64_t W, uint8_t* nanflag, unsigned long long* stats) {
    const BoxDenom denom = box_reciprocal(box_denominator(rad));
    const size_t lds = boxx_lds_bytes(NTI, L, rad);
// ... 175 lines not shown
static TileRoute pick_tile_route(const Run& r, bool packed) {
    const Plan& pl = r.pl;
    static const bool no_tile = is1(getenv("TRI_NO_TILE_MEDREJ"));
    const int T = (int)pl.T, G = (int)pl.G;
    const size_t wsA = 2 * (size_t)pl.PT * pl.Fa, wsB = (size_t)pl.PF * T;
    const size_t mr_nb = (size_t)pl.maxchunk * T;
    TileRoute t = {false, (mr_nb / 4) & ~(size_t)3, (mr_nb / 8) & ~(size_t)3, 0};
    for (int g = 0; g < G; g++) t.ytiles += (int)cdiv(r.p->chunk_ends[g + 1] - r.p->chunk_ends[g], 64);
    t.use = pl.vec && wsB % 4 == 0 && wsA % 4 == 0 && packed && !no_fused_reject() && !no_tile && !fused_medrej() && G <= 65535 &&
            mrt_scratch_words(G, t.ccap, t.ucap) <= wsA && (medrej_force_fallback() || (pl.maxchunk - 1) * (int64_t)T >= 65536) &&
            t.ytiles > 0 && t.ytiles <= 65535;
    return t;
}
static unsigned medrej_capq(size_t wsA, int G) {
    const size_t per_block = (wsA / (size_t)G) & ~(size_t)7;
    return (unsigned)std::min<size_t>(per_block / 2, 0x3ffffffcu);
}

struct BgStep {
    int r0, r1;
    bool final_pass;
    TimeStage time;
    bool time_needs_bytes;
    bool time_defers;
    FreqPick freq;
    bool freq_transposes;
    Reject reject;
    bool reads_ft_flags;
};

static BgStep pick_bg_step(const Run& r, bool packed, bool tile_route, int ext) {
    const Plan& pl = r.pl;
    const int T = (int)pl.T, Fa = (int)pl.Fa, G = (int)pl.G;
    const size_t wsA = 2 * (size_t)pl.PT * Fa, wsB = (size_t)pl.PF * T;
    BgStep s;
    s.final_pass = ext == 0;
    const double e = (double)(s.final_pass ? 1 : ext);
    s.r0 = (int)box_radius(e * r.p->spike_width_time);
    s.r1 = (int)box_radius(e * r.p->spike_width_freq);

    static const bool prebuild = [] { const char* e = getenv("TRI_TIME_PREBUILD"); return !(e && e[0] == '0'); }();
    const bool sweep = s.r0 > 0 && colfilter_lds_block(s.r0, Fa) > 0;
    if (s.r0 == 0) s.time = TimeStage::BuildOnly;
    else if (sweep && packed) s.time = TimeStage::PackedSweep;
    else if (sweep && prebuild) {
        static const bool want_direct = is1(getenv("TRI_FILTER_DIRECT_FT"));
        s.time = (want_direct && T % 4 == 0 && wsB % 4 == 0) ? TimeStage::PrebuiltDirectFT : TimeStage::Prebuilt;
    } else s.time = TimeStage::ByteFlags;
    s.time_needs_bytes = packed && (s.time == TimeStage::BuildOnly || s.time == TimeStage::ByteFlags);

    s.freq = s.time == TimeStage::PrebuiltDirectFT ? pick_freq_unfused(s.r1, T)
                                                   : pick_freq_stage(s.r1, Fa, T, (size_t)(r.ws.Ao - r.ws.Aw), !r.ampl_cached || r.data_mask);
    s.freq_transposes = s.time != TimeStage::PrebuiltDirectFT;
    s.time_defers = s.freq.route == FreqStage::Transposed;

    static const bool no_tfr = is1(getenv("TRI_FILTER_NO_TF_REJECT"));
    const bool vec4 = pl.vec && wsB % 4 == 0;
    if (s.final_pass) s.reject = Reject::None;
    else if (s.freq.route == FreqStage::ExactRows && packed && !no_tfr && G <= 65535 && (uint64_t)T * Fa * 4u < (1ull << 31))
        s.reject = Reject::InRows;
    else if (tile_route) s.reject = Reject::Tile;
    else if (vec4 && wsA % 4 == 0 && packed && !no_fused_reject() && fused_medrej() && medrej_capq(wsA, G) >= 1024 && G <= 65535 &&
             (uint64_t)T * Fa * 4u < (1ull << 32))
        s.reject = Reject::OnePass;
    else if (vec4 && packed && !no_fused_reject()) s.reject = Reject::MedianReject4T;
    else s.reject = vec4 ? Reject::MedianReject4 : Reject::MedianReject;
    s.reads_ft_flags = s.time_needs_bytes || (!s.final_pass && s.reject != Reject::InRows);
    return s;
}

struct BgImages {
    int T, Fa;
    int64_t W;
    const float *dataTF, *dataFT;
    const uint8_t* flagsTF;
    uint8_t* comb;
    float *Aw, *Ao; size_t wsA;
    float *Bw, *Bo; size_t wsB;
    float* rows; size_t ws_rows;
    const uint8_t* mask; size_t ws_mask;
    uint8_t* nanflag;
    float* residP;
    unsigned long long* xstats;
};

struct BgState {
    uint8_t *cur_ft, *alt_ft;
    bool bgf_ft_stale;
    bool wrote_panel;
};

static int bg_time_stage(const Run& r, const BgStep& s, const BgImages& im, const BgState& st, float* den_t) {
    const int T = im.T, Fa = im.Fa;
    const size_t N = (size_t)T * Fa;
    const int64_t W = im.W;
    int rc = TRI_OK;
    *den_t = 0.0f;
    float* const defer = s.time_defers ? den_t : nullptr;
    const uint8_t* fl = im.flagsTF;
    if (s.time_needs_bytes) {
        rc = launch_transpose<uint8_t>(r, st.cur_ft, im.comb, Fa, T, N, N, W);
        if (rc) return rc;
        fl = im.comb;
    }
    switch (s.time) {
        case TimeStage::BuildOnly:
            hipLaunchKernelGGL(k_build_wo, grid1(N, W), dim3(256), 0, r.st, im.dataTF, fl, im.Aw, im.Ao, N, N, im.wsA);
            LAUNCHCHK();
            return TRI_OK;
        case TimeStage::PackedSweep:
            return launch_colfilter(r, ColSrc::PackedFlags, im.Aw, im.Ao, im.dataTF, fl, im.Aw, im.Ao, T, Fa, s.r0, im.wsA, N, im.wsA, W, COL_WEIGHTS_01, defer);
        case TimeStage::Prebuilt:
        case TimeStage::PrebuiltDirectFT:
            if (N % 4 == 0 && im.wsA % 4 == 0)
                hipLaunchKernelGGL(k_build_wo4, grid1(N / 4, W), dim3(256), 0, r.st, im.dataTF, fl, im.Aw, im.Ao, N / 4, N, im.wsA);
            else
                hipLaunchKernelGGL(k_build_wo, grid1(N, W), dim3(256), 0, r.st, im.dataTF, fl, im.Aw, im.Ao, N, N, im.wsA);
            LAUNCHCHK();
            if (s.time == TimeStage::Prebuilt)
                return launch_colfilter(r, ColSrc::Images, im.Aw, im.Ao, nullptr, nullptr, im.Aw, im.Ao, T, Fa, s.r0, im.wsA, 0, im.wsA, W, COL_WEIGHTS_01, defer);
            return launch_colfilter(r, ColSrc::Images, im.Aw, im.Ao, nullptr, nullptr, im.Bw + s.freq.off, im.Bo + s.freq.off, T, Fa, s.r0, im.wsA, 0, im.wsB, W, COL_TRANSPOSED_OUT);
        case TimeStage::ByteFlags:
            return launch_colfilter(r, ColSrc::ByteFlags, im.Aw, im.Ao, im.dataTF, fl, im.Aw, im.Ao, T, Fa, s.r0, im.wsA, N, im.wsA, W);
    }
    return set_err(TRI_EINVAL, "internal: no such time stage");
}

template <int MODE>
static int bg_freq_stage_mode(const Run& r, const BgStep& s, const BgImages& im, BgState& st, float den_t) {
    const int T = im.T, Fa = im.Fa, r1 = s.r1;
    const size_t N = (size_t)T * Fa, wsA = im.wsA, wsB = im.wsB;
    const int64_t W = im.W;
    uint8_t* const nan = MODE == 2 ? im.nanflag : nullptr;
    float den_f = 0.0f;
    int rc = TRI_OK;
    if (MODE == 2) HIPCHK(hipMemsetAsync(im.nanflag, 0, (size_t)W * T, r.st));
    switch (s.freq.route) {
        case FreqStage::ExactRows:
            rc = launch_boxx<MODE>(r, s.freq.xl, im.Aw, im.Ao, im.dataTF, im.mask, im.rows, MODE == 2 ? im.Aw : nullptr, Fa, T, Fa, r1, wsA, N,
                                   im.ws_mask, im.ws_rows, MODE == 2 ? wsA : 0, W, nan, im.xstats);
            if (!rc && MODE == 2) rc = launch_transpose<float>(r, im.Aw, im.Bw, T, Fa, wsA, wsB, W);
            if (rc || s.reject == Reject::InRows) return rc;
            return launch_transpose<float>(r, im.rows, im.Bo, T, Fa, im.ws_rows, wsB, W);
        case FreqStage::FusedRing:
            return launch_boxf<MODE>(r, s.freq.ks, im.Aw, im.Ao, im.Bw, im.Bo, im.dataFT, Fa, T, Fa, r1, wsA, wsB, N, W, nan,
                                     MODE == 2 ? im.residP : nullptr, MODE == 2 ? N : 0, &st.wrote_panel);
        case FreqStage::FusedLds:
            return launch_colfilter_tf<MODE>(r, im.Aw, im.Ao, im.Bw, im.Bo, im.dataFT, Fa, T, Fa, r1, wsA, wsB, N, W, nan);
        case FreqStage::LdsDiv:
            rc = launch_colfilter_t(r, im.Aw, im.Ao, im.Bw, im.Bo, Fa, T, Fa, r1, wsA, wsB, W, &den_f);
            break;
        case FreqStage::Lane4Div:
            rc = launch_colfilter_t4(r, im.Aw, im.Ao, im.Bw, im.Bo, Fa, T, Fa, r1, wsA, wsB, W, &den_f);
            break;
        case FreqStage::Transposed:
            if (s.freq_transposes) {
                rc = launch_transpose<float>(r, im.Aw, im.Bw + s.freq.off, T, Fa, wsA, wsB, W, den_t);
                if (!rc) rc = launch_transpose<float>(r, im.Ao, im.Bo + s.freq.off, T, Fa, wsA, wsB, W, den_t);
            }
            if (!rc && r1 > 0) rc = launch_colfilter(r, ColSrc::Images, im.Bw, im.Bo, nullptr, nullptr, im.Bw, im.Bo, Fa, T, r1, wsB, 0, wsB, W, 0, &den_f);
            break;
    }
    if (rc) return rc;
    return launch_masked_div<MODE>(r, im.Bw, im.Bo, im.dataFT, N, wsB, N, W, den_f, nan, MODE == 2 ? T : 1);
}
static int bg_freq_stage(const Run& r, const BgStep& s, const BgImages& im, BgState& st, float den_t) {
    return s.final_pass ? bg_freq_stage_mode<2>(r, s, im, st, den_t) : bg_freq_stage_mode<1>(r, s, im, st, den_t);
}

static int bg_reject_stage(const Run& r, const BgStep& s, const TileRoute& tile, bool packed, BgState& st) {
    const Plan& pl = r.pl;
    const Ws& ws = r.ws;
    const int T = (int)pl.T, Fa = (int)pl.Fa, G = (int)pl.G;
    const int64_t W = r.Wb;
    const size_t N = (size_t)T * Fa, wsA = 2 * (size_t)pl.PT * Fa, wsB = (size_t)pl.PF * T;
    const double rej = TRI_MAD_NORMAL * r.p->background_reject;
    if (s.reject == Reject::None) return TRI_OK;
    if (s.reject != Reject::Tile && st.cur_ft == ws.flagsFT)
        return set_err(TRI_EUNSUPPORTED, "internal: background flags read in place on a route that rewrites them");
    switch (s.reject) {
        case Reject::InRows: {
            unsigned* gc = reinterpret_cast<unsigned*>(ws.Aw);
            unsigned cap = (unsigned)(std::min<size_t>((wsA / 2) / (size_t)G, 0x7fffffffu) & ~(size_t)3);
            if (median_no_predict() || (int64_t)cap < pl.maxchunk * pl.T || wsA % 4 != 0) { gc = nullptr; cap = 0; }
            hipLaunchKernelGGL((k_median2<false, true>), dim3((unsigned)G, (unsigned)W), dim3(256), 0, r.st, (const float*)ws.Ao,
                               (const uint8_t*)ws.bgfTF, ws.med, wsA, N, (size_t)0, (size_t)1, ws.segC_start, ws.segC_len, 1, G,
                               gc, gc ? wsA : (size_t)0, cap, T / 4, Fa);
            hipLaunchKernelGGL(k_reject_tf, dim3((unsigned)cdiv(Fa, 256), (unsigned)(T / 4), (unsigned)W), dim3(256), 0, r.st,
                               (const float*)ws.Ao, reinterpret_cast<unsigned*>(ws.bgfTF), ws.med, ws.d_chunk_of, rej, T / 4, Fa, Fa, G,
                               wsA, N / 4);
            LAUNCHCHK();
            st.bgf_ft_stale = true;
            return TRI_OK;
        }
        case Reject::Tile: {
            unsigned* sc = reinterpret_cast<unsigned*>(ws.Aw);
            hipLaunchKernelGGL(k_mr_predict, dim3((unsigned)G, (unsigned)W), dim3(256), 0, r.st, (const float*)ws.Bo, (const uint8_t*)st.cur_ft,
                               ws.d_chunk_ends, rej, T / 4, G, wsB, N, sc, wsA, tile.ccap, tile.ucap, medrej_force_fallback());
            for (unsigned round = 1; round <= 2; round++) {
                hipLaunchKernelGGL(k_mr_pass, dim3((unsigned)cdiv(T / 4, 64), (unsigned)tile.ytiles, (unsigned)W), dim3(256), 0, r.st, (const float*)ws.Bo,
                                   (const uint8_t*)st.cur_ft, st.alt_ft, ws.bgfTF, ws.d_chunk_ends, Fa, T / 4, G, wsB, N, sc, wsA, tile.ccap, tile.ucap, round);
                hipLaunchKernelGGL(k_mr_finish, dim3((unsigned)G, (unsigned)W), dim3(256), 0, r.st, (const float*)ws.Bo, (const uint8_t*)st.cur_ft, st.alt_ft,
                                   ws.bgfTF, ws.med, ws.d_chunk_ends, rej, Fa, T / 4, G, wsB, N, sc, wsA, tile.ccap, tile.ucap, round);
            }
            hipLaunchKernelGGL(k_median_reject, dim3((unsigned)G, (unsigned)W), dim3(256), 0, r.st, (const float*)ws.Bo, (const uint8_t*)st.cur_ft,
                               st.alt_ft, ws.bgfTF, ws.med, ws.d_chunk_ends, rej, Fa, T / 4, G, wsB, N, sc, wsA, 0u, 0u, 1,
                               (const unsigned*)sc, wsA, (int)MRT_PARW, 11);
            LAUNCHCHK();
            std::swap(st.cur_ft, st.alt_ft);
            if (st.alt_ft == ws.flagsFT) st.alt_ft = ws.fflFT;
            return TRI_OK;
        }
        case Reject::OnePass: {
            const unsigned capq = medrej_capq(wsA, G);
            hipLaunchKernelGGL(k_median_reject, dim3((unsigned)G, (unsigned)W), dim3(256), 0, r.st, (const float*)ws.Bo, (const uint8_t*)st.cur_ft,
                               st.alt_ft, ws.bgfTF, ws.med, ws.d_chunk_ends, rej, Fa, T / 4, G, wsB, N,
                               reinterpret_cast<unsigned*>(ws.Aw), wsA, capq, capq, medrej_force_fallback());
            LAUNCHCHK();
            std::swap(st.cur_ft, st.alt_ft);
            return TRI_OK;
        }
        default:
            break;
    }
    MedianJob j;
    j.data = ws.Bo; j.flags = st.cur_ft; j.med = ws.med; j.WSd = wsB; j.WSf = N;
    j.seg_start = ws.segB_start; j.seg_len = ws.segB_len; j.R = 1; j.G = G; j.W = W; j.max_len = pl.maxchunk * pl.T;
    j.vec_ok = T % 4 == 0 && wsB % 4 == 0 && N % 4 == 0;
    j.gcand = reinterpret_cast<unsigned*>(ws.Aw); j.cand_ws = wsA;
    j.cand_cap = (unsigned)(std::min<size_t>(wsA / (size_t)G, 0x7fffffffu) & ~(size_t)3);
    const int rc = launch_median(r, j);
    if (rc) return rc;
    if (s.reject == Reject::MedianReject4T) {
        hipLaunchKernelGGL(k_reject4_t, dim3((unsigned)cdiv(T / 4, 64), (unsigned)cdiv(Fa, 64), (unsigned)W), dim3(64, 4), 0, r.st,
                           ws.Bo, st.cur_ft, ws.bgfTF, ws.med, ws.d_chunk_of, rej, Fa, T / 4, G, wsB, N);
        LAUNCHCHK();
        return TRI_OK;
    }
    if (s.reject == Reject::MedianReject4)
        hipLaunchKernelGGL(k_reject4, grid1(N / 4, W), dim3(256), 0, r.st, ws.Bo, st.cur_ft, ws.med, ws.d_chunk_of, rej, T / 4, G, N / 4, wsB, N);
    else
        hipLaunchKernelGGL(k_reject<true>, grid1(N, W), dim3(256), 0, r.st, ws.Bo, st.cur_ft, ws.med, ws.d_chunk_of, rej, Fa, T, G, wsB, N);
    LAUNCHCHK();
    if (packed) return launch_transpose<float>(r, reinterpret_cast<const float*>(st.cur_ft), reinterpret_cast<float*>(ws.bgfTF), Fa, T / 4, N / 4, N / 4, W);
    return launch_transpose<uint8_t>(r, st.cur_ft, ws.bgfTF, Fa, T, N, N, W);
}

int background2d(const Run& r, bool flagsFT_current, float* residP = nullptr, bool* wroteP = nullptr) {
    const Plan& pl = r.pl;
    const Ws& ws = r.ws;
    const int T = (int)pl.T, Fa = (int)pl.Fa;
    const int64_t W = r.Wb;
    const size_t N = (size_t)T * Fa;
    const bool packed = bg_flags_packed(T, N);
    const TileRoute tile = pick_tile_route(r, packed);
    static const bool copy_flags = is1(getenv("TRI_BG_COPY_FLAGS"));
    bool flags_in_place = flagsFT_current && !copy_flags && packed && tile.use;
    for (int ext = pl.nit; ext >= 1 && flags_in_place; ext--)
        if (pick_bg_step(r, packed, tile.use, ext).freq.route == FreqStage::ExactRows) flags_in_place = false;
    int rc = TRI_OK;
    if (!flags_in_place)
        rc = flagsFT_current ? launch_u8<0>(r, ws.flagsFT, ws.bgfFT, N, N, N, W)
                             : launch_transpose<uint8_t>(r, ws.flagsTF, ws.bgfFT, T, Fa, N, N, W);
    if (rc) return rc;
    if (packed)
        rc = launch_transpose<float>(r, reinterpret_cast<const float*>(flags_in_place ? ws.flagsFT : ws.bgfFT), reinterpret_cast<float*>(ws.bgfTF), Fa, T / 4, N / 4, N / 4, W);
    else
        rc = launch_u8<0>(r, ws.flagsTF, ws.bgfTF, N, N, N, W);
    if (rc) return rc;

    BgImages im;
    im.T = T; im.Fa = Fa; im.W = W;
    im.dataTF = ws.dataTF; im.dataFT = ws.dataFT;
    im.flagsTF = ws.bgfTF; im.comb = ws.comb;
    im.Aw = ws.Aw; im.Ao = ws.Ao; im.wsA = 2 * (size_t)pl.PT * Fa;
    im.Bw = ws.Bw; im.Bo = ws.Bo; im.wsB = (size_t)pl.PF * T;
    im.rows = ws.Ao; im.ws_rows = im.wsA;
    im.mask = r.ampl_cached ? r.data_mask : nullptr; im.ws_mask = r.data_mask_ws;
    im.nanflag = reinterpret_cast<uint8_t*>(ws.rowcnt);
    im.residP = residP; im.xstats = nullptr;
    BgState st = {flags_in_place ? ws.flagsFT : ws.bgfFT, flags_in_place ? ws.bgfFT : ws.fflFT, false, false};
    for (int ext = pl.nit; ext >= 0; ext--) {
        const BgStep s = pick_bg_step(r, packed, tile.use, ext);
        if (st.bgf_ft_stale && s.reads_ft_flags) {
            rc = launch_transpose<float>(r, reinterpret_cast<const float*>(ws.bgfTF), reinterpret_cast<float*>(st.cur_ft), T / 4, Fa, N / 4, N / 4, W);
            if (rc) return rc;
            st.bgf_ft_stale = false;
        }
        float den_t = 0.0f;
        rc = bg_time_stage(r, s, im, st, &den_t);
        if (!rc) rc = bg_freq_stage(r, s, im, st, den_t);
        if (!rc) rc = bg_reject_stage(r, s, tile, packed, st);
        if (rc) return rc;
    }
    if (wroteP) *wroteP = st.wrote_panel;
    return launch_interp(r, ws.Bo, Fa, T, im.wsB, W, reinterpret_cast<const uint8_t*>(ws.rowcnt), (const float*)ws.dataFT, N, ws.Bw,
                         st.wrote_panel ? residP : nullptr, N);
}


enum class Begin {
    FusedCached,
    Cached,
    Prepare4,
    Prepare
};
enum class SpecOr {
    Scalar,
    Rows16,
    FtInPlace,
    FtInPlaceDeferTf
};
enum class ChunkFlags {
    ExtraSources,
    OrMore16,
    OrBytes
};
enum class Finish {
    FusedDilate,
    Combine16Dilate,
    Combine16,
    Combine
};
enum class FinalKernel {
    NanMask16,
    Vis16,
    Scalar
};
struct IterStep {
    Begin begin; SpecOr spec_or; ChunkFlags chunk_flags; Finish finish; FinalKernel final_kernel;
    bool panel;
    bool fused_resid;
    int lo, hi, flo, fhi;
    bool ft_current() const { return spec_or == SpecOr::FtInPlace || spec_or == SpecOr::FtInPlaceDeferTf; }
};

static void smear_extents(int64_t e, int* lo, int* hi) {
    const int64_t half = e >= 0 ? e / 2 : -((-e + 1) / 2);
    *lo = (int)-half; *hi = (int)(-half + e);
}
static bool st_no_panel() { static const bool off = is1(getenv("TRI_ST_NO_PANEL")); return off; }

static IterStep pick_iteration(const Run& r) {
    const Plan& pl = r.pl;
    const int T = (int)pl.T, F = (int)pl.F, Fa = (int)pl.Fa;
    const size_t N = (size_t)T * Fa;
    static const bool no_fused_begin = is1(getenv("TRI_NO_FUSED_BEGIN"));
    static const bool no_ft_or = is1(getenv("TRI_NO_FT_SPEC_OR"));
    static const bool no_fused_or = is1(getenv("TRI_NO_FUSED_OR"));
    static const bool no_fused_dilate = is1(getenv("TRI_NO_FUSED_DILATE"));
    static const bool no_fused_resid = [] { const char* e = getenv("TRI_NO_FUSED_RESID_TF"); return !(e && e[0] == '0'); }();
    IterStep s;
    smear_extents(r.p->time_extend, &s.lo, &s.hi);
    smear_extents(r.p->freq_extend, &s.flo, &s.fhi);
    if (!r.ampl_cached) s.begin = pl.vec ? Begin::Prepare4 : Begin::Prepare;
    else s.begin = (!no_fused_begin && T % 4 == 0 && Fa % 4 == 0 && N % 4 == 0 && (uintptr_t)r.ws.iter % 4 == 0) ? Begin::FusedCached : Begin::Cached;
    if (!pl.vec) s.spec_or = SpecOr::Scalar;
    else if (no_ft_or || T % 16 != 0) s.spec_or = SpecOr::Rows16;
    else s.spec_or = bg_flags_packed(T, N) ? SpecOr::FtInPlaceDeferTf : SpecOr::FtInPlace;
    const bool defer_tf = s.spec_or == SpecOr::FtInPlaceDeferTf;
    if (defer_tf && !no_fused_or && median_takes_extra_flags(pl.maxchunk) && Fa % 4 == 0) s.chunk_flags = ChunkFlags::ExtraSources;
    else s.chunk_flags = defer_tf ? ChunkFlags::OrMore16 : ChunkFlags::OrBytes;
    if (!pl.vec) s.finish = Finish::Combine;
    else if (s.flo != -1 || s.fhi != 2) s.finish = Finish::Combine16;
    else s.finish = no_fused_dilate ? Finish::Combine16Dilate : Finish::FusedDilate;
    s.final_kernel = !pl.vec ? FinalKernel::Scalar : r.ampl_cached ? FinalKernel::NanMask16 : FinalKernel::Vis16;
    s.panel = !st_no_panel() && s.chunk_flags == ChunkFlags::ExtraSources && s.finish == Finish::FusedDilate && Fa % 64 == 0 && Fa == F &&
              median_takes_extra_flags(pl.maxchunk + 3) && st_use_fused(pl.swT) && st_use_mask(T, Fa);
    s.fused_resid = s.panel && !no_fused_resid;
    return s;
}

template <int VD>
static int launch_prepare(const Run& r, const IterStep& s, const void* vis) {
    const Plan& pl = r.pl;
    const Ws& ws = r.ws;
    const size_t N = (size_t)pl.T * pl.Fa, W = (size_t)r.Wb;
    if (s.begin == Begin::Prepare4)
        hipLaunchKernelGGL(k_prepare4<VD>, dim3((unsigned)cdiv(N * W / 4, 256)), dim3(256), 0, r.st, vis, ws.iter, ws.dataTF, ws.flagsTF, N * W / 4);
    else
        hipLaunchKernelGGL(k_prepare<VD>, grid1(N, W), dim3(256), 0, r.st, vis, ws.iter, ws.dataTF, ws.flagsTF, (int)pl.T, (int)pl.F, (int)pl.Fa, (int)pl.avg);
    LAUNCHCHK();
    return TRI_OK;
}
template <int VD>
static int launch_final(const Run& r, const IterStep& s, const void* vis, uint8_t* out_flags, bool update_iter) {
    const Ws& ws = r.ws;
    const int T = (int)r.pl.T, F = (int)r.pl.F, upd = update_iter ? 1 : 0;
    const size_t NF = (size_t)T * F, W = (size_t)r.Wb;
    const double row_limit = r.p->flag_all_freq_frac * (double)F, col_limit = (double)T * r.p->flag_all_time_frac;
    if (s.final_kernel == FinalKernel::NanMask16)
        hipLaunchKernelGGL(k_final16<TRI_VIS_NANMASK>, grid1(NF / 16, W), dim3(256), 0, r.st, ws.dil, ws.rowcnt, ws.colcnt, (const void*)ws.nanmask, out_flags, ws.iter, T, F / 16, row_limit, col_limit, upd);
    else if (s.final_kernel == FinalKernel::Vis16)
        hipLaunchKernelGGL(k_final16<VD>, grid1(NF / 16, W), dim3(256), 0, r.st, ws.dil, ws.rowcnt, ws.colcnt, vis, out_flags, ws.iter, T, F / 16, row_limit, col_limit, upd);
    else
        hipLaunchKernelGGL(k_final<VD>, grid1(NF, W), dim3(256), 0, r.st, ws.dil, ws.rowcnt, ws.colcnt, vis, out_flags, ws.iter, T, F, row_limit, col_limit, upd);
    LAUNCHCHK();
    return TRI_OK;
}
#define BY_VIS_DTYPE(FN, ...) \
    (vis_dtype == TRI_VIS_C64 ? FN<TRI_VIS_C64>(__VA_ARGS__) : vis_dtype == TRI_VIS_F64 ? FN<TRI_VIS_F64>(__VA_ARGS__) : FN<TRI_VIS_F32>(__VA_ARGS__))

static int iter_begin(const Run& r, const IterStep& s, const void* vis, int vis_dtype) {
    const Ws& ws = r.ws;
    const int T = (int)r.pl.T, Fa = (int)r.pl.Fa;
    const size_t N = (size_t)T * Fa;
    const int64_t W = r.Wb;
    int rc = TRI_OK;
    switch (s.begin) {
        case Begin::FusedCached:
            hipLaunchKernelGGL((k_transpose_u8w<true, true>), dim3((unsigned)cdiv(Fa, 64), (unsigned)cdiv(T, 128), (unsigned)W), dim3(256), 0, r.st,
                               ws.iter, ws.flagsFT, ws.flagsTF, ws.dataFT, T, Fa, N, N, N, N);
            break;
        case Begin::Cached:
            rc = launch_u8<0>(r, ws.iter, ws.flagsTF, N, N, N, W);
            if (!rc) rc = launch_transpose<uint8_t>(r, ws.flagsTF, ws.flagsFT, T, Fa, N, N, W);
            if (rc) return rc;
            hipLaunchKernelGGL(k_zero_flagged4, grid1(N / 4, W), dim3(256), 0, r.st, ws.flagsFT, ws.dataFT, N / 4, N, N);
            break;
        case Begin::Prepare4:
        case Begin::Prepare:
            rc = BY_VIS_DTYPE(launch_prepare, r, s, vis);
            if (!rc) rc = launch_transpose<float>(r, ws.dataTF, ws.dataFT, T, Fa, N, N, W);
            if (!rc) rc = launch_transpose<uint8_t>(r, ws.flagsTF, ws.flagsFT, T, Fa, N, N, W);
            return rc;
    }
    LAUNCHCHK();
    return TRI_OK;
}

static int time_medians(const Run& r, const float* dataFT, size_t ws_data) {
    const Ws& ws = r.ws;
    const int T = (int)r.pl.T, Fa = (int)r.pl.Fa;
    MedianJob j;
    j.data = dataFT; j.flags = ws.flagsFT; j.med = ws.med; j.WSd = ws_data; j.WSf = (size_t)T * Fa; j.RS = (size_t)T;
    j.seg_start = ws.segT_start; j.seg_len = ws.segT_len; j.R = Fa; j.G = 1; j.W = r.Wb; j.max_len = r.pl.T;
    j.rows_aligned = T % 4 == 0; j.segs_aligned = true;
    return launch_median(r, j);
}

static int iter_spectrum(const Run& r, const IterStep& s) {
    const Ws& ws = r.ws;
    const int T = (int)r.pl.T, Fa = (int)r.pl.Fa, Wn = (int)r.Wb;
    const size_t N = (size_t)T * Fa, nS = (size_t)Fa * Wn;
    const int64_t W = r.Wb;
    int rc = time_medians(r, ws.dataFT, N);
    if (rc) return rc;
    hipLaunchKernelGGL(k_spec_from_med, dim3((unsigned)cdiv(nS, 256)), dim3(256), 0, r.st, ws.med, ws.sdata, ws.sflags, Fa, Wn);
    LAUNCHCHK();
    rc = spectrum_background(r);
    if (!rc) rc = launch_sub(r, ws.sdata, ws.so, ws.sres, nS, 0, 0, 0, 1);
    if (!rc) rc = spectrum_medians(r, ws.sres, ws.sflags);
    if (!rc) rc = launch_colst(r, r.pl.swF, ws.sres, ws.smed, ws.sout, ws.d_chunk_ends, Fa, Wn, (int)r.pl.G, 0, 0, 1);
    if (rc) return rc;
    if (s.spec_or != SpecOr::Scalar)
        hipLaunchKernelGGL(k_spec_rows, dim3((unsigned)cdiv(nS, 256)), dim3(256), 0, r.st, ws.sout, ws.srows, Fa, Wn);
    switch (s.spec_or) {
        case SpecOr::Scalar:
            hipLaunchKernelGGL(k_or_spec, grid1(N, W), dim3(256), 0, r.st, ws.flagsTF, ws.sout, T, Fa, Wn);
            break;
        case SpecOr::Rows16:
            hipLaunchKernelGGL(k_or_spec16, grid1(N / 16, W), dim3(256), 0, r.st, ws.flagsTF, ws.srows, T, Fa / 16);
            break;
        case SpecOr::FtInPlace:
            hipLaunchKernelGGL(k_or_spec16, grid1(N / 16, W), dim3(256), 0, r.st, ws.flagsTF, ws.srows, T, Fa / 16);
            hipLaunchKernelGGL(k_or_spec_ft16, grid1(N / 16, W), dim3(256), 0, r.st, ws.flagsFT, ws.srows, T / 16, Fa);
            break;
        case SpecOr::FtInPlaceDeferTf:
            hipLaunchKernelGGL(k_or_spec_ft16, grid1(N / 16, W), dim3(256), 0, r.st, ws.flagsFT, ws.srows, T / 16, Fa);
            break;
    }
    LAUNCHCHK();
    return TRI_OK;
}

static int iter_residual(const Run& r, const IterStep& s, const float** residTF) {
    const Ws& ws = r.ws;
    const int T = (int)r.pl.T, Fa = (int)r.pl.Fa;
    bool wrote_panel = false;
    const int rc = background2d(r, s.ft_current(), s.fused_resid ? ws.residP : nullptr, &wrote_panel);
    *residTF = wrote_panel ? ws.residP : ws.Aw;
    if (rc || wrote_panel) return rc;
    return launch_transpose<float>(r, ws.Bw, ws.Aw, Fa, T, (size_t)r.pl.PF * T, (size_t)T * Fa, r.Wb, 0.0f, s.panel);
}

static int iter_sumthreshold(const Run& r, const IterStep& s, const float* residTF) {
    const Plan& pl = r.pl;
    const Ws& ws = r.ws;
    const int T = (int)pl.T, Fa = (int)pl.Fa, G = (int)pl.G;
    const size_t N = (size_t)T * Fa, wsB = (size_t)pl.PF * T;
    const int64_t W = r.Wb;
    int rc = s.ft_current() ? TRI_OK : launch_transpose<uint8_t>(r, ws.flagsTF, ws.flagsFT, T, Fa, N, N, W);
    if (!rc) rc = time_medians(r, ws.Bw, wsB);
    if (!rc) rc = launch_colst(r, pl.swT, residTF, ws.med, ws.tflTF, ws.d_tends, T, Fa, 1, N, N, W, s.panel);
    if (rc) return rc;
    MedianJob cj;
    cj.data = residTF; cj.flags = ws.flagsTF; cj.med = ws.med; cj.WSd = cj.WSf = N; cj.RS = (size_t)Fa;
    cj.seg_start = ws.segC_start; cj.seg_len = ws.segC_len; cj.R = T; cj.G = G; cj.W = W; cj.max_len = pl.maxchunk;
    cj.rows_aligned = Fa % 4 == 0;
    switch (s.chunk_flags) {
        case ChunkFlags::ExtraSources:
            cj.flags2 = ws.tflTF; cj.colflags = ws.srows; cj.WScol = (size_t)Fa; cj.panel_rows = s.panel ? T : 0;
            break;
        case ChunkFlags::OrMore16:
            hipLaunchKernelGGL(k_or_spec_more16, grid1(N / 16, W), dim3(256), 0, r.st, ws.flagsTF, ws.srows, ws.tflTF, T, Fa / 16);
            LAUNCHCHK();
            break;
        case ChunkFlags::OrBytes:
            rc = launch_u8<1>(r, ws.tflTF, ws.flagsTF, N, N, N, W);
            break;
    }
    if (!rc) rc = launch_median(r, cj);
    if (!rc) rc = launch_colst(r, pl.swF, ws.Bw, ws.med, ws.fflFT, ws.d_chunk_ends, Fa, T, G, wsB, N, W);
    if (!rc) rc = launch_transpose<uint8_t>(r, ws.fflFT, ws.fflTF, Fa, T, N, N, W);
    return rc;
}

static int iter_taps(const Run& r, const IterStep& s, const float* residTF) {
    const Ws& ws = r.ws;
    const int T = (int)r.pl.T, Fa = (int)r.pl.Fa, Wn = (int)r.Wb;
    const size_t N = (size_t)T * Fa;
    const Debug& d = *r.dbg;
    hipLaunchKernelGGL(k_gather_col_f32, dim3((unsigned)cdiv(Fa, 256)), dim3(256), 0, r.st, ws.sres, d.f32, Fa, Wn, 0);
    hipLaunchKernelGGL(k_gather_col_u8, dim3((unsigned)cdiv(Fa, 256)), dim3(256), 0, r.st, ws.sout, d.u8, Fa, Wn, 0);
    if (s.panel) {
        hipLaunchKernelGGL(k_unpanel<float>, dim3((unsigned)cdiv(N, 256)), dim3(256), 0, r.st, residTF, d.f32 + Fa + N, T, Fa);
        hipLaunchKernelGGL(k_unpanel<uint8_t>, dim3((unsigned)cdiv(N, 256)), dim3(256), 0, r.st, (const uint8_t*)ws.tflTF, d.u8 + Fa, T, Fa);
    } else {
        HIPCHK(hipMemcpyAsync(d.f32 + Fa + N, residTF, N * sizeof(float), hipMemcpyDeviceToDevice, r.st));
        HIPCHK(hipMemcpyAsync(d.u8 + Fa, ws.tflTF, N, hipMemcpyDeviceToDevice, r.st));
    }
    LAUNCHCHK();
    HIPCHK(hipMemcpyAsync(d.f32 + Fa, ws.Bo, N * sizeof(float), hipMemcpyDeviceToDevice, r.st));
    HIPCHK(hipMemcpyAsync(d.u8 + Fa + N, ws.fflTF, N, hipMemcpyDeviceToDevice, r.st));
    return TRI_OK;
}

static int iter_finish(const Run& r, const IterStep& s, const void* vis, int vis_dtype, uint8_t* out_flags, bool update_iter) {
    const Ws& ws = r.ws;
    const int T = (int)r.pl.T, F = (int)r.pl.F, Fa = (int)r.pl.Fa, Wn = (int)r.Wb;
    const size_t N = (size_t)T * Fa;
    const int64_t W = r.Wb;
    const dim3 grid16((unsigned)cdiv(F / 16, 64), (unsigned)T, (unsigned)W);
    HIPCHK(hipMemsetAsync(ws.rowcnt, 0, (size_t)W * T * sizeof(int), r.st));
    switch (s.finish) {
        case Finish::FusedDilate:
            if (s.panel) hipLaunchKernelGGL(k_combine_dilate16<true>, grid16, dim3(64), 0, r.st, ws.srows, ws.tflTF, ws.fflTF, ws.dil, ws.rowcnt, T, F / 16, s.lo, s.hi);
            else hipLaunchKernelGGL(k_combine_dilate16<false>, grid16, dim3(64), 0, r.st, ws.srows, ws.tflTF, ws.fflTF, ws.dil, ws.rowcnt, T, F / 16, s.lo, s.hi);
            hipLaunchKernelGGL(k_colcount, grid1(F / 4, W), dim3(256), 0, r.st, ws.dil, ws.colcnt, T, F / 4);
            break;
        case Finish::Combine16Dilate:
            hipLaunchKernelGGL(k_combine16, grid1(N / 16, W), dim3(256), 0, r.st, ws.srows, ws.tflTF, ws.fflTF, ws.comb, T, Fa / 16, s.lo, s.hi);
            hipLaunchKernelGGL((k_unaverage16<-1, 3>), grid16, dim3(64), 0, r.st, ws.comb, ws.dil, ws.rowcnt, T, F / 16);
            hipLaunchKernelGGL(k_colcount, grid1(F / 4, W), dim3(256), 0, r.st, ws.dil, ws.colcnt, T, F / 4);
            break;
        case Finish::Combine16:
        case Finish::Combine:
            if (s.finish == Finish::Combine16)
                hipLaunchKernelGGL(k_combine16, grid1(N / 16, W), dim3(256), 0, r.st, ws.srows, ws.tflTF, ws.fflTF, ws.comb, T, Fa / 16, s.lo, s.hi);
            else
                hipLaunchKernelGGL(k_combine, grid1(N, W), dim3(256), 0, r.st, ws.sout, ws.tflTF, ws.fflTF, ws.comb, T, Fa, Wn, s.lo, s.hi);
            LAUNCHCHK();
            HIPCHK(hipMemsetAsync(ws.colcnt, 0, (size_t)W * F * sizeof(int), r.st));
// ... 390 lines not shown
                                             (int)ntime, terms, vw, flag_windows);                                   \
            else if (fl)  hipLaunchKernelGGL((k_pack_scan_rows_v<NC, S, false, true>), grid, dim3(256), 0, st, d, m, \
                                             fl, src_row, src_rows, row_bl, row_time, e0, (int)nchan, (int)nbl,      \
                                             (int)ntime, terms, vw, flag_windows);                                   \
            else          hipLaunchKernelGGL((k_pack_scan_rows_v<NC, S, false, false>), grid, dim3(256), 0, st, d,   \
                                             m, fl, src_row, src_rows, row_bl, row_time, e0, (int)nchan, (int)nbl,   \
                                             (int)ntime, terms, vw, flag_windows);                                   \
        } while (0)
        if (vec && ncorr == 4 && stokes) TRI_PACK_SCAN_ROWS_V(4, true);
        else if (vec && ncorr == 4) TRI_PACK_SCAN_ROWS_V(4, false);
        else if (vec && ncorr == 2 && stokes) TRI_PACK_SCAN_ROWS_V(2, true);
        else if (vec && ncorr == 2) TRI_PACK_SCAN_ROWS_V(2, false);
        else if (vec && ncorr == 1 && stokes) TRI_PACK_SCAN_ROWS_V(1, true);
        else if (vec && ncorr == 1) TRI_PACK_SCAN_ROWS_V(1, false);
        else
            hipLaunchKernelGGL(k_pack_scan_rows, grid, dim3(256), 0, st, d, m, fl, src_row, src_rows, row_bl, row_time,
                               e0, (int)nchan, (int)ncorr, (int)nbl, (int)ntime, stokes ? 1 : 0, terms, vw,
                               flag_windows);
#undef TRI_PACK_SCAN_ROWS_V
    });
}

extern "C" int tri_unpack_scan_rows(const uint8_t* flag_windows, const int64_t* dst_row, int64_t out_rows,
                                    const int32_t* row_bl, const int32_t* row_time, int64_t n, int64_t nchan,
                                    int64_t wcorr, int64_t out_ncorr, int64_t nbl, int64_t ntime, uint8_t* out_flags,
                                    void* stream) {
    if (!flag_windows || !row_bl || !row_time || !out_flags) return set_err(TRI_EINVAL, "NULL pointer argument");
    if (n < 0 || out_rows < 0 || nchan <= 0 || out_ncorr <= 0 || nbl < 0 || ntime < 0)
        return set_err(TRI_EINVAL, "bad shape");
    if (wcorr != 1 && wcorr != out_ncorr) return set_err(TRI_EINVAL, "wcorr must be 1 or out_ncorr");
    if (!dst_row && n > out_rows) return set_err(TRI_EINVAL, "a list without dst_row writes rows [0, n): n > out_rows");
    hipStream_t st = (hipStream_t)stream;
    return for_row_slabs(n, nchan, out_ncorr, nbl, ntime, [&](int64_t e0, unsigned nr) {
        const dim3 grid((unsigned)cdiv(nchan, 256), nr, 1);
        if (out_ncorr == 4 && (uintptr_t)out_flags % 4 == 0)
            hipLaunchKernelGGL(k_unpack_scan_rows<4>, grid, dim3(256), 0, st, flag_windows, dst_row, out_rows, row_bl,
                               row_time, e0, (int)nchan, (int)wcorr, 4, (int)nbl, (int)ntime, out_flags);
        else
            hipLaunchKernelGGL(k_unpack_scan_rows<0>, grid, dim3(256), 0, st, flag_windows, dst_row, out_rows, row_bl,
                               row_time, e0, (int)nchan, (int)wcorr, (int)out_ncorr, (int)nbl, (int)ntime, out_flags);
    });
}

extern "C" int tri_bench_reject(const float* resid, const uint8_t* flags_in, uint8_t* flags_out, uint8_t* flags_t4, double* med,
                                int64_t n_win, int64_t n_chan, int64_t n_time, const int64_t* chunk_ends, int64_t n_chunk_ends,
                                double reject, int repeats, float* ms_per_step, void* stream) {
    if (!resid || !flags_in || !flags_out || !flags_t4 || !med || !chunk_ends || !ms_per_step) return set_err(TRI_EINVAL, "NULL pointer argument");
    if (n_win <= 0 || n_win > 65535 || n_chan <= 0 || n_time <= 0 || n_time % 4 != 0 || n_chunk_ends < 2 || n_chunk_ends > 256 || repeats <= 0)
        return set_err(TRI_EINVAL, "bad shape");
    if ((uint64_t)n_chan * (uint64_t)n_time * 4u >= (1ull << 31)) return set_err(TRI_EUNSUPPORTED, "a window of 2^31 bytes or more");
    const int G = (int)n_chunk_ends - 1, T = (int)n_time, Fa = (int)n_chan;
    int64_t maxchunk = 0, minchunk = n_chan;
    int ytiles = 0;
    for (int g = 0; g < G; g++) {
        const int64_t c = chunk_ends[g + 1] - chunk_ends[g];
        if (c <= 0 || chunk_ends[g] < 0 || chunk_ends[g + 1] > n_chan) return set_err(TRI_EINVAL, "bad chunk");
        maxchunk = std::max(maxchunk, c); minchunk = std::min(minchunk, c);
        ytiles += (int)cdiv(c, 64);
    }
    if (chunk_ends[0] != 0 || chunk_ends[G] != n_chan) return set_err(TRI_EINVAL, "chunks must cover the channels");
    if (minchunk * (int64_t)T < 65536 || ytiles > 65535) return set_err(TRI_EUNSUPPORTED, "blocks below 65536 samples take the two-kernel route");
    hipStream_t st = (hipStream_t)stream;
    const size_t N = (size_t)Fa * T;
    const size_t nb = (size_t)maxchunk * T, ccap = (nb / 4) & ~(size_t)3, ucap = (nb / 8) & ~(size_t)3;
    const size_t wsS = mrt_scratch_words(G, ccap, ucap);
    DevBuf<unsigned> scb;
    DevBuf<int64_t> endsb;
    HIPCHK(scb.alloc((size_t)n_win * wsS));
    HIPCHK(endsb.alloc((size_t)n_chunk_ends));
    unsigned* sc = scb.get();
    int64_t* d_ends = endsb.get();
    HIPCHK(hipMemcpyAsync(d_ends, chunk_ends, (size_t)n_chunk_ends * sizeof(int64_t), hipMemcpyHostToDevice, st));
    HIPCHK(hipStreamSynchronize(st));
    const double rej = TRI_MAD_NORMAL * reject;
    HipEvent e0, e1;
    HIPCHK(hipEventCreate(e0.out()));
    HIPCHK(hipEventCreate(e1.out()));
    const unsigned W = (unsigned)n_win;
    HIPCHK(hipEventRecord(e0.get(), st));
    for (int i = 0; i < repeats; i++) {
        hipLaunchKernelGGL(k_mr_predict, dim3((unsigned)G, W), dim3(256), 0, st, resid, flags_in, d_ends, rej, T / 4, G, N, N, sc, wsS, ccap, ucap, 0);
        for (unsigned round = 1; round <= 2; round++) {
            hipLaunchKernelGGL(k_mr_pass, dim3((unsigned)cdiv(T / 4, 64), (unsigned)ytiles, W), dim3(256), 0, st, resid, flags_in, flags_out, flags_t4,
                               d_ends, Fa, T / 4, G, N, N, sc, wsS, ccap, ucap, round);
            hipLaunchKernelGGL(k_mr_finish, dim3((unsigned)G, W), dim3(256), 0, st, resid, flags_in, flags_out, flags_t4, med, d_ends, rej, Fa, T / 4, G,
                               N, N, sc, wsS, ccap, ucap, round);
        }
        hipLaunchKernelGGL(k_median_reject, dim3((unsigned)G, W), dim3(256), 0, st, resid, flags_in, flags_out, flags_t4, med, d_ends, rej, Fa, T / 4, G,
                           N, N, sc, wsS, 0u, 0u, 1, (const unsigned*)sc, wsS, (int)MRT_PARW, 11);
    }
    HIPCHK(hipEventRecord(e1.get(), st));
    hipError_t le = hipGetLastError();
    hipError_t se = hipEventSynchronize(e1.get());
    float ms = 0.f;
    if (le == hipSuccess && se == hipSuccess) (void)hipEventElapsedTime(&ms, e0.get(), e1.get());
    if (le != hipSuccess) return set_err(TRI_EHIP, "launch: %s", hipGetErrorString(le));
    if (se != hipSuccess) return set_err(TRI_EHIP, "sync: %s", hipGetErrorString(se));
    *ms_per_step = ms / (float)repeats;
    return TRI_OK;
}

static int st_hook(const float* data, const double* mad, uint8_t* out, int64_t n_win, int64_t n_line, int64_t n_col,
                   const int64_t* windows, int64_t n_windows, double outlier_nsigma, double rho, int variant, int repeats,
                   float* ms_per_launch, void* stream, const int64_t* chunk_ends, int64_t n_chunk_ends, bool flagger_pick) {
    if (!data || !mad || !out || !windows || !ms_per_launch || !chunk_ends) return set_err(TRI_EINVAL, "NULL pointer argument");
    if (n_win <= 0 || n_line <= 0 || n_col <= 0 || repeats <= 0 || n_win > 65535) return set_err(TRI_EINVAL, "bad shape");
    if (n_chunk_ends < 2 || n_chunk_ends > 256) return set_err(TRI_EINVAL, "2 .. 256 chunk ends");
    for (int64_t g = 0; g < n_chunk_ends; g++)
        if (chunk_ends[g] < 0 || chunk_ends[g] > n_line || (g > 0 && chunk_ends[g] < chunk_ends[g - 1]))
            return set_err(TRI_EINVAL, "chunk ends must not decrease and must lie in [0, n_line]");
    const int G = (int)n_chunk_ends - 1;
    const int64_t o0 = chunk_ends[0], o1 = chunk_ends[G];
    hipStream_t st = (hipStream_t)stream;
    StWin sw;
    int rc = make_stwin(windows, n_windows, rho, &sw);
    if (rc) return rc;
    double thr_scale = outlier_nsigma * TRI_MAD_NORMAL;
    size_t nthreads = (size_t)n_win * n_col * G;
    int C = (int)n_col, L = (int)n_line;
    bool can_fuse = sw.nw == 4 && sw.w[0] == 1 && sw.w[1] == 2 && sw.w[2] == 4 && sw.w[3] == 8;
    if ((variant == 2 || variant == 3) && !can_fuse) return set_err(TRI_EUNSUPPORTED, "register cascade needs windows (1,2,4,8)");
    if (variant == 3 && !((uint64_t)L * (uint64_t)C * 4u < (1ull << 31)))
        return set_err(TRI_EUNSUPPORTED, "lane-mask cascade needs a window below 2^31 bytes");
    if (variant == 5 && !(can_fuse && C % 64 == 0 && (uint64_t)L * (uint64_t)C * 4u < (1ull << 31)))
        return set_err(TRI_EUNSUPPORTED, "panel SumThreshold: windows (1,2,4,8), a multiple of 64 columns, a window below 2^31 bytes");
    if (variant == 5 && G > 1) return set_err(TRI_EUNSUPPORTED, "panel SumThreshold: one chunk only (launch_colst never pairs a panel with chunks)");
    if (variant == 0 && can_fuse) variant = st_use_mask(L, C) ? ((G == 1 && C % 64 == 0 && !st_no_panel()) ? 5 : 3) : 2;
    if (variant == 0 && flagger_pick && st_use_pipe(sw)) variant = 4;
    if (variant == 4) {
        if (sw.nw > 8 || stp_lds_bytes(sw) > 160 * 1024) return set_err(TRI_EUNSUPPORTED, "stage pipeline: more than eight windows, or the flag ring does not fit LDS");
        HIPCHK(lds_optin_all(160 * 1024, &k_colst_pipe));
    }
    DevBuf<double> ring;
    DevBuf<uint8_t> acc;
    DevBuf<int64_t> d_ends;
    HIPCHK(ring.alloc(nthreads * sw.ringtot));
    HIPCHK(acc.alloc(nthreads * sw.acccap));
    HIPCHK(d_ends.alloc((size_t)n_chunk_ends));
    HIPCHK(hipMemcpyAsync(d_ends.get(), chunk_ends, (size_t)n_chunk_ends * sizeof(int64_t), hipMemcpyHostToDevice, st));
    HIPCHK(hipStreamSynchronize(st));
    HipEvent e0, e1;
    HIPCHK(hipEventCreate(e0.out()));
    HIPCHK(hipEventCreate(e1.out()));
    size_t ws = (size_t)n_line * n_col;
    DevBuf<float> pdata;
    DevBuf<uint8_t> pout;
    if (variant == 5) {
        HIPCHK(pdata.alloc((size_t)n_win * ws));
        HIPCHK(pout.alloc((size_t)n_win * ws));
        {
            ScopedSet<bool> pause(g_klog_on, false);
            hipLaunchKernelGGL(k_panelize<float>, dim3((unsigned)cdiv((int64_t)ws, 256), (unsigned)n_win), dim3(256), 0, st, data, pdata.get(), L, C, ws);
        }
        LAUNCHCHK();
    }
    const StKernel k = variant == 5 ? StKernel::MaskPanel : variant == 3 ? StKernel::Mask : variant == 2 ? StKernel::Fused :
                       variant == 4 ? StKernel::Pipe : StKernel::Dyn;
    const float* kdata = variant == 5 ? (const float*)pdata.get() : data;
    uint8_t* kout = variant == 5 ? pout.get() : out;
    HIPCHK(hipEventRecord(e0.get(), st));
    for (int i = 0; i < repeats; i++) {
        rc = st_launch(st, k, sw, kdata, mad, kout, d_ends.get(), thr_scale, L, C, G, ws, ws, n_win, ring.get(), acc.get());
        if (rc) return rc;
    }
    HIPCHK(hipEventRecord(e1.get(), st));
    HIPCHK(hipEventSynchronize(e1.get()));
    LAUNCHCHK();
// ... 531 lines not shown
```

Baseline: 3101 Mvis/s.

## Skip loads and stores for fully-flagged dead channels in background filter

```diff
diff --git a/tricolour_amd/csrc/kernels_boxline.hpp b/tricolour_amd/csrc/kernels_boxline.hpp
--- a/tricolour_amd/csrc/kernels_boxline.hpp
+++ b/tricolour_amd/csrc/kernels_boxline.hpp
@@ -222,6 +222,9 @@
 #endif
 __host__ __device__ constexpr int boxf_nsub(int ks) { return (BOXF_DOUBLE_STAGE && ks <= 16 && boxr_pf_f(ks) == 16) ? 2 : 1; }
 #define BOXF_TS 34
+#ifndef BOXF_SKIP_DEAD
+#define BOXF_SKIP_DEAD 0
+#endif
 #ifndef BOXF_STREAM_AUX
 #define BOXF_STREAM_AUX 0
 #endif
@@ -234,6 +237,7 @@
        uint8_t* __restrict__ nanflag, float* __restrict__ dstP, size_t pws) {
     extern __shared__ float cf_ring[];
     constexpr int PF = boxr_pf_f(KS);
+    static_assert(PF <= 32, "dead-channel mask: one bit per position of a block");
     static_assert(MODE != 2 || (PF / 2) % 4 == 0, "panel output: groups of four positions per lane");
     constexpr int NSUB = boxf_nsub(KS);
     constexpr int PL = PF * NSUB;
@@ -299,17 +303,30 @@
     const int hoff = (colok ? c : 0) * 4 + (int)((unsigned)hrow * rowb);
     const float* eb = tiles + (size_t)hrow * TS + hl;
     float dpre[PF / 2];
+    constexpr int OOBL = 0x7ffffff0;
+    unsigned dnext = 0, dm = 0;
+    auto lookup = [&](int m0) {
+        if constexpr (MODE == 1 && BOXF_SKIP_DEAD != 0) {
+            if (nanflag != nullptr) {
+                const int i = m0 - 3 - 4 * r + lane;
+                const bool in = lane < PF && i >= 0 && i < n;
+                const size_t e = win * (size_t)n + (size_t)(in ? i : 0);
+                dnext = in ? (unsigned)nanflag[e] : 0u;
+            }
+        }
+    };
     auto issue_data = [&](int m0, bool fast) {
         const int i0 = m0 - 3 - 4 * r;
         if (fast) {
 #pragma unroll
             for (int k = 0; k < PF / 2; k++)
-                dpre[k] = __builtin_bit_cast(float, __builtin_amdgcn_raw_buffer_load_b32(xrs, hoff, (int)((unsigned)(i0 + k) * rowb), BOXF_STREAM_AUX));
+                dpre[k] = __builtin_bit_cast(float, __builtin_amdgcn_raw_buffer_load_b32(xrs, (MODE == 1 && BOXF_SKIP_DEAD != 0 && ((dm >> k) & 1u)) ? OOBL : hoff, (int)((unsigned)(i0 + k) * rowb), BOXF_STREAM_AUX));
         } else {
 #pragma unroll
             for (int k = 0; k < PF / 2; k++) {
                 const int i = i0 + hrow + k;
-                const bool ok = i >= 0 && i < n;
+                bool ok = i >= 0 && i < n;
+                if constexpr (MODE == 1 && BOXF_SKIP_DEAD != 0) ok = ok && !((dm >> k) & 1u);
                 const float v = __builtin_bit_cast(float, __builtin_amdgcn_raw_buffer_load_b32(xrs, ok ? (colok ? c : 0) * 4 + (int)((unsigned)i * rowb) : 0, 0, 0));
                 dpre[k] = ok ? v : 0.0f;
             }
@@ -323,6 +340,7 @@
     const int total = n + 4 * r + 3;
     bool line_nan = false;
     issue(0);
+    lookup(0);
     for (int mb = 0; mb < total; mb += UNR) {
 #pragma unroll
         for (int b = 0; b < UNR / PF; b++) {
@@ -337,6 +355,10 @@
                     issue(m0 + PL);
                 }
                 const bool fast = m0 >= 4 * r + 3 && m0 + PF <= n;
+                if constexpr (MODE == 1 && BOXF_SKIP_DEAD != 0) {
+                    dm = (unsigned)__builtin_amdgcn_ballot_w64(dnext != 0u) >> hrow;
+                    lookup(m0 + PF);
+                }
                 issue_data(m0, fast);
                 float xin = tile[ro * TS + hl];
                 if (fast) {
@@ -380,7 +402,7 @@
                                 const int vo = fast ? hoff : (c * 4 + (int)((unsigned)i * rowb));
                                 const int so = fast ? (int)((unsigned)(i0 + k) * rowb) : 0;
                                 if (MODE == 1) {
-                                    __builtin_amdgcn_raw_buffer_store_b32(__builtin_bit_cast(unsigned, fabsf(dpre[k] - bg)), ors, vo, so, BOXF_STREAM_AUX);
+                                    __builtin_amdgcn_raw_buffer_store_b32(__builtin_bit_cast(unsigned, fabsf(dpre[k] - bg)), ors, (BOXF_SKIP_DEAD != 0 && ((dm >> k) & 1u)) ? OOBL : vo, so, BOXF_STREAM_AUX);
                                 } else {
                                     __builtin_amdgcn_raw_buffer_store_b32(__builtin_bit_cast(unsigned, bg), ors, vo, so, BOXF_STREAM_AUX);
                                     res[MODE == 2 ? k : 0] = dpre[k] - bg;
diff --git a/tricolour_amd/csrc/kernels_boxpipe.hpp b/tricolour_amd/csrc/kernels_boxpipe.hpp
--- a/tricolour_amd/csrc/kernels_boxpipe.hpp
+++ b/tricolour_amd/csrc/kernels_boxpipe.hpp
@@ -373,6 +373,10 @@
 __host__ __device__ constexpr int boxqf_prefetch8(int nblk) {
     return nblk == 6 ? 3 : (nblk == 8 ? 4 : (nblk == 9 ? 3 : (nblk == 10 ? BOXQF_P10 : (nblk == 12 ? 4 : nblk))));
 }
+#ifndef BOXQF_SKIP_DEAD
+#define BOXQF_SKIP_DEAD 1
+#endif
+#define BOXQF_DEAD_MAX_N 8192
 #ifndef BOXQF_MINW8
 #define BOXQF_MINW8 4
 #endif
@@ -452,11 +456,35 @@
     const __amdgpu_buffer_rsrc_t ors = __builtin_amdgcn_make_buffer_rsrc((void*)(dstO + win * dws), 0, (int)((unsigned)n * rowb), 0x00020000);
     const __amdgpu_buffer_rsrc_t wrs = __builtin_amdgcn_make_buffer_rsrc((void*)(dstW + win * dws), 0, (int)((unsigned)n * rowb), 0x00020000);
     float dpre[P][FN];
+    unsigned* const dbits = reinterpret_cast<unsigned*>(cf_ring + boxqf_lds_floats(B, DBL));
+    bool has_dead = false;
+    if constexpr (MODE == 1 && BOXQF_SKIP_DEAD != 0) {
+        has_dead = nanflag != nullptr;
+        if (has_dead) {
+            const unsigned* t32 = reinterpret_cast<const unsigned*>(nanflag) + win * (size_t)(n / 4);
+            for (int k = tid; k < (n + 31) / 32; k += 512) {
+                unsigned m = 0;
+#pragma unroll
+                for (int j = 0; j < 8; j++) {
+                    const int e = 32 * k + 4 * j;
+                    const unsigned w4 = e < n ? t32[e >> 2] : 0u;
+                    m |= (((w4 & 0xFFu) ? 1u : 0u) | ((w4 & 0xFF00u) ? 2u : 0u) | ((w4 & 0xFF0000u) ? 4u : 0u) | ((w4 & 0xFF000000u) ? 8u : 0u)) << (4 * j);
+                }
+                dbits[k] = m;
+            }
+            __syncthreads();
+        }
+    }
+    auto live = [&](int i) -> bool {
+        if constexpr (MODE == 1 && BOXQF_SKIP_DEAD != 0) { if (has_dead) return !((dbits[i >> 5] >> (i & 31)) & 1u); }
+        return true;
+    };
     auto issue_data = [&](int blk, int q) {
 #pragma unroll
         for (int h = 0; h < FN; h++) {
             const int i = blk * B + f_u + 8 * h - 4 * r;
-            const bool ok = blk >= 0 && i >= 0 && i < n && colok;
+            bool ok = blk >= 0 && i >= 0 && i < n && colok;
+            if constexpr (MODE == 1 && BOXQF_SKIP_DEAD != 0) { if (blk >= 0 && i >= 0 && i < n) ok = ok && live(blk * B + wave + 8 * h - 4 * r); }
             dpre[q][h] = __builtin_bit_cast(float, __builtin_amdgcn_raw_buffer_load_b32(xrs, (int)(ok ? (unsigned)i * rowb + coff : OOB), 0, 0));
         }
     };
@@ -572,7 +600,8 @@
 #pragma unroll
                 for (int h = 0; h < FN; h++) {
                     const int i = bs * B + f_u + 8 * h - 4 * r;
-                    const bool ok = bs >= 0 && bs < NB && i >= 0 && i < n && colok;
+                    bool ok = bs >= 0 && bs < NB && i >= 0 && i < n && colok;
+                    if constexpr (MODE == 1 && BOXQF_SKIP_DEAD != 0) { if (bs >= 0 && i >= 0 && i < n) ok = ok && live(bs * B + wave + 8 * h - 4 * r); }
                     const unsigned off = ok ? (unsigned)i * rowb + coff : OOB;
                     const float bg = (wq[h] == 0.0f) ? NAN : oq[h] / wq[h];
                     const float dv = dpre[q][h];
diff --git a/tricolour_amd/csrc/kernels_elementwise.hpp b/tricolour_amd/csrc/kernels_elementwise.hpp
--- a/tricolour_amd/csrc/kernels_elementwise.hpp
+++ b/tricolour_amd/csrc/kernels_elementwise.hpp
@@ -82,7 +82,8 @@
 template <bool COPY, bool ZERO>
 __global__ __launch_bounds__(256) void k_transpose_u8w(const uint8_t* __restrict__ src, uint8_t* __restrict__ dst,
                                                        uint8_t* __restrict__ copy, float* __restrict__ data, int R, int C,
-                                                       size_t src_ws, size_t dst_ws, size_t copy_ws, size_t data_ws) {
+                                                       size_t src_ws, size_t dst_ws, size_t copy_ws, size_t data_ws,
+                                                       uint8_t* __restrict__ dead = nullptr) {
     __shared__ unsigned tile[128][17];
     const uint8_t* s = src + (size_t)blockIdx.z * src_ws;
     uint8_t* d = dst + (size_t)blockIdx.z * dst_ws;
@@ -119,6 +120,10 @@
             const int c = c0 + 4 * q + b;
             if (c >= C) break;
             *reinterpret_cast<unsigned*>(d + (size_t)c * R + r) = o[b];
+            if (dead) {
+                const unsigned long long live = __builtin_amdgcn_ballot_w64(((o[b] - 0x01010101u) & ~o[b] & 0x80808080u) != 0u);
+                if (bx == 0 && ((live >> (tid & 32)) & 0xFFFFFFFFull)) dead[(size_t)blockIdx.z * C + c] = 0;
+            }
             if (ZERO && o[b]) {
                 const unsigned f = o[b];
                 float4* pd = reinterpret_cast<float4*>(data + (size_t)blockIdx.z * data_ws + (size_t)c * R + r);
@@ -522,11 +527,13 @@
     else *pb = make_uint4(nz_bytes(va.x), nz_bytes(va.y), nz_bytes(va.z), nz_bytes(va.w));
 }
 
-__global__ void k_spec_rows(const uint8_t* __restrict__ spec, uint8_t* __restrict__ rows, int Fa, int Wn) {
+__global__ void k_spec_rows(const uint8_t* __restrict__ spec, uint8_t* __restrict__ rows, int Fa, int Wn, uint8_t* __restrict__ dead = nullptr) {
     size_t i = (size_t)blockIdx.x * blockDim.x + threadIdx.x;
     if (i >= (size_t)Fa * Wn) return;
     int w = (int)(i / Fa), f = (int)(i % Fa);
-    rows[i] = spec[(size_t)f * Wn + w];
+    const uint8_t v = spec[(size_t)f * Wn + w];
+    rows[i] = v;
+    if (dead && v) dead[i] = 1;
 }
 
 __global__ void k_or_spec16(uint8_t* __restrict__ flags, const uint8_t* __restrict__ spec_rows, int T, int Fa16) {
diff --git a/tricolour_amd/csrc/kernels_reject_tile.hpp b/tricolour_amd/csrc/kernels_reject_tile.hpp
--- a/tricolour_amd/csrc/kernels_reject_tile.hpp
+++ b/tricolour_amd/csrc/kernels_reject_tile.hpp
@@ -163,7 +163,8 @@
 __global__ void __launch_bounds__(256, MRT_PASS_WAVES)
 k_mr_pass(const float* __restrict__ resid, const uint8_t* __restrict__ flags_in, uint8_t* __restrict__ flags_out,
           uint8_t* __restrict__ flags_t4, const int64_t* __restrict__ chunk_ends, int L, int C4, int G,
-          size_t ws_resid, size_t ws_flags, unsigned* __restrict__ gscratch, size_t scratch_ws, size_t ccap, size_t ucap, unsigned round) {
+          size_t ws_resid, size_t ws_flags, unsigned* __restrict__ gscratch, size_t scratch_ws, size_t ccap, size_t ucap, unsigned round,
+          const uint8_t* __restrict__ dead = nullptr) {
     __shared__ unsigned hist[SEL_BINS + 64];
     __shared__ unsigned tile[64][65];
     __shared__ unsigned lcand[4][MRT_WCAND];
@@ -183,6 +184,8 @@
         }
         if (g >= G) return;
     }
+    uint8_t dead_row = 0;
+    if (dead && l0 + lane < c1) dead_row = dead[win * (size_t)L + (size_t)(l0 + lane)];
     const MrtLayout lay{gscratch + win * scratch_ws, G, ccap, ucap};
     MrtPar* par = lay.par(g);
     __shared__ unsigned sh_status;
@@ -206,8 +209,15 @@
     for (int q = 0; q < 16; q++) {
         const int l = l0 + ty + 4 * q;
         const size_t i = (l < c1 && w < C4) ? (size_t)l * C4 + w : (size_t)l0 * C4;
-        rv[q] = r4[i];
         f[q] = fin[i];
+    }
+    const unsigned long long deadm = __builtin_amdgcn_ballot_w64(dead_row != 0);
+#pragma unroll
+    for (int q = 0; q < 16; q++) {
+        const int l = l0 + ty + 4 * q;
+        const size_t i = (l < c1 && w < C4) ? (size_t)l * C4 + w : (size_t)l0 * C4;
+        rv[q] = make_float4(0.0f, 0.0f, 0.0f, 0.0f);
+        if (!((deadm >> (ty + 4 * q)) & 1ull)) rv[q] = r4[i];
     }
     __syncthreads();
     unsigned mb1 = 0;
diff --git a/tricolour_amd/csrc/tricolour_amd.hip b/tricolour_amd/csrc/tricolour_amd.hip
--- a/tricolour_amd/csrc/tricolour_amd.hip
+++ b/tricolour_amd/csrc/tricolour_amd.hip
@@ -164,6 +164,7 @@
     uint8_t *iter, *flagsTF, *flagsFT, *bgfTF, *bgfFT, *tflTF, *fflFT, *fflTF, *comb, *dil;
     float* residP;
     int *rowcnt, *colcnt;
+    uint8_t* dead;
     double* med;
     float *sdata, *sw, *so, *sres;
     uint8_t *sflags, *sbgf, *sout, *srows;
@@ -215,6 +216,7 @@
     ws->residP = dry ? nullptr : reinterpret_cast<float*>(ws->bgfTF);
     ws->rowcnt = b.get<int>(W * T);
     ws->colcnt = b.get<int>(W * F);
+    ws->dead = reinterpret_cast<uint8_t*>(ws->colcnt);
     ws->nanmask = b.get<uint16_t>(W * N / 16 + 8);
     ws->itab = b.get<int>(3 * W * (size_t)cdiv(Fa, INTERP_SEG) * std::max<size_t>(T, 1));
     ws->med = b.get<double>(W * std::max(Fa, T * G));
@@ -861,7 +863,7 @@
         ((uintptr_t)src % 4 == 0) && ((uintptr_t)dst % 4 == 0)) {
         dim3 gridw((unsigned)cdiv(C, 64), (unsigned)cdiv(R, 128), (unsigned)W);
         hipLaunchKernelGGL((k_transpose_u8w<false, false>), gridw, dim3(256), 0, r.st, (const uint8_t*)src, (uint8_t*)dst,
-                           (uint8_t*)nullptr, (float*)nullptr, R, C, sws, dws, (size_t)0, (size_t)0);
+                           (uint8_t*)nullptr, (float*)nullptr, R, C, sws, dws, (size_t)0, (size_t)0, (uint8_t*)nullptr);
         LAUNCHCHK();
         return TRI_OK;
     }
@@ -983,7 +985,9 @@
     HIPCHK(lds_optin_all(160 * 1024, &k_boxqf<KS, MODE, B>));
     const BoxDenom denom = box_reciprocal(box_denominator(rad));
     dim3 grid((unsigned)cdiv(C, 64), (unsigned)W);
-    hipLaunchKernelGGL((k_boxqf<KS, MODE, B>), grid, dim3(512), boxqf_lds_bytes(B, boxqf_dbl(KS, B)), r.st, srcW, gap, dstW, dstO, data, n, C, ld, rad,
+    if (MODE == 1 && n > BOXQF_DEAD_MAX_N) nanflag = nullptr;
+    const size_t dead_lds = (MODE == 1 && nanflag) ? (size_t)cdiv(n, 32) * 4 : 0;
+    hipLaunchKernelGGL((k_boxqf<KS, MODE, B>), grid, dim3(512), boxqf_lds_bytes(B, boxqf_dbl(KS, B)) + dead_lds, r.st, srcW, gap, dstW, dstO, data, n, C, ld, rad,
                        denom, sws_img, dws, ws_data, nanflag);
     LAUNCHCHK();
     return TRI_OK;
@@ -992,7 +996,8 @@
 template <int MODE>
 int launch_boxf(const Run& r, int ks, const float* srcW, const float* srcO, float* dstW, float* dstO, const float* data,
                 int n, int C, int ld, int rad, size_t sws_img, size_t dws, size_t ws_data, int64_t W, uint8_t* nanflag,
-                float* dstP = nullptr, size_t pws = 0, bool* wroteP = nullptr) {
+                float* dstP = nullptr, size_t pws = 0, bool* wroteP = nullptr, const uint8_t* dead = nullptr) {
+    if (MODE == 1) nanflag = const_cast<uint8_t*>(dead);
     if (MODE != 2 || n % 64 != 0) dstP = nullptr;
     {
         static const bool off = is1(getenv("TRI_FILTER_NO_PIPE_F"));
@@ -1334,6 +1339,7 @@
     uint8_t* nanflag;
     float* residP;
     unsigned long long* xstats;
+    const uint8_t* dead;
 };
 
 struct BgState {
@@ -1396,7 +1402,7 @@
             return launch_transpose<float>(r, im.rows, im.Bo, T, Fa, im.ws_rows, wsB, W);
         case FreqStage::FusedRing:
             return launch_boxf<MODE>(r, s.freq.ks, im.Aw, im.Ao, im.Bw, im.Bo, im.dataFT, Fa, T, Fa, r1, wsA, wsB, N, W, nan,
-                                     MODE == 2 ? im.residP : nullptr, MODE == 2 ? N : 0, &st.wrote_panel);
+                                     MODE == 2 ? im.residP : nullptr, MODE == 2 ? N : 0, &st.wrote_panel, MODE == 1 ? im.dead : nullptr);
         case FreqStage::FusedLds:
             return launch_colfilter_tf<MODE>(r, im.Aw, im.Ao, im.Bw, im.Bo, im.dataFT, Fa, T, Fa, r1, wsA, wsB, N, W, nan);
         case FreqStage::LdsDiv:
@@ -1420,7 +1426,7 @@
     return s.final_pass ? bg_freq_stage_mode<2>(r, s, im, st, den_t) : bg_freq_stage_mode<1>(r, s, im, st, den_t);
 }
 
-static int bg_reject_stage(const Run& r, const BgStep& s, const TileRoute& tile, bool packed, BgState& st) {
+static int bg_reject_stage(const Run& r, const BgStep& s, const BgImages& im, const TileRoute& tile, bool packed, BgState& st) {
     const Plan& pl = r.pl;
     const Ws& ws = r.ws;
     const int T = (int)pl.T, Fa = (int)pl.Fa, G = (int)pl.G;
@@ -1451,7 +1457,7 @@
                                ws.d_chunk_ends, rej, T / 4, G, wsB, N, sc, wsA, tile.ccap, tile.ucap, medrej_force_fallback());
             for (unsigned round = 1; round <= 2; round++) {
                 hipLaunchKernelGGL(k_mr_pass, dim3((unsigned)cdiv(T / 4, 64), (unsigned)tile.ytiles, (unsigned)W), dim3(256), 0, r.st, (const float*)ws.Bo,
-                                   (const uint8_t*)st.cur_ft, st.alt_ft, ws.bgfTF, ws.d_chunk_ends, Fa, T / 4, G, wsB, N, sc, wsA, tile.ccap, tile.ucap, round);
+                                   (const uint8_t*)st.cur_ft, st.alt_ft, ws.bgfTF, ws.d_chunk_ends, Fa, T / 4, G, wsB, N, sc, wsA, tile.ccap, tile.ucap, round, im.dead);
                 hipLaunchKernelGGL(k_mr_finish, dim3((unsigned)G, (unsigned)W), dim3(256), 0, r.st, (const float*)ws.Bo, (const uint8_t*)st.cur_ft, st.alt_ft,
                                    ws.bgfTF, ws.med, ws.d_chunk_ends, rej, Fa, T / 4, G, wsB, N, sc, wsA, tile.ccap, tile.ucap, round);
             }
@@ -1498,7 +1504,7 @@
     return launch_transpose<uint8_t>(r, st.cur_ft, ws.bgfTF, Fa, T, N, N, W);
 }
 
-int background2d(const Run& r, bool flagsFT_current, float* residP = nullptr, bool* wroteP = nullptr) {
+int background2d(const Run& r, bool flagsFT_current, float* residP = nullptr, bool* wroteP = nullptr, bool have_dead = false) {
     const Plan& pl = r.pl;
     const Ws& ws = r.ws;
     const int T = (int)pl.T, Fa = (int)pl.Fa;
@@ -1531,6 +1537,8 @@
     im.mask = r.ampl_cached ? r.data_mask : nullptr; im.ws_mask = r.data_mask_ws;
     im.nanflag = reinterpret_cast<uint8_t*>(ws.rowcnt);
     im.residP = residP; im.xstats = nullptr;
+    const bool use_dead = have_dead && flags_in_place;
+    im.dead = use_dead ? ws.dead : nullptr;
     BgState st = {flags_in_place ? ws.flagsFT : ws.bgfFT, flags_in_place ? ws.bgfFT : ws.fflFT, false, false};
     for (int ext = pl.nit; ext >= 0; ext--) {
         const BgStep s = pick_bg_step(r, packed, tile.use, ext);
@@ -1542,7 +1550,7 @@
         float den_t = 0.0f;
         rc = bg_time_stage(r, s, im, st, &den_t);
         if (!rc) rc = bg_freq_stage(r, s, im, st, den_t);
-        if (!rc) rc = bg_reject_stage(r, s, tile, packed, st);
+        if (!rc) rc = bg_reject_stage(r, s, im, tile, packed, st);
         if (rc) return rc;
     }
     if (wroteP) *wroteP = st.wrote_panel;
@@ -1623,6 +1631,11 @@
     return s;
 }
 
+#ifndef BG_DEAD_CHANNELS
+#define BG_DEAD_CHANNELS 1
+#endif
+static bool iter_builds_dead(const IterStep& s) { return BG_DEAD_CHANNELS && s.begin == Begin::FusedCached && s.ft_current(); }
+
 template <int VD>
 static int launch_prepare(const Run& r, const IterStep& s, const void* vis) {
     const Plan& pl = r.pl;
@@ -1661,8 +1674,9 @@
     int rc = TRI_OK;
     switch (s.begin) {
         case Begin::FusedCached:
+            if (iter_builds_dead(s)) HIPCHK(hipMemsetAsync(ws.dead, 1, (size_t)W * Fa, r.st));
             hipLaunchKernelGGL((k_transpose_u8w<true, true>), dim3((unsigned)cdiv(Fa, 64), (unsigned)cdiv(T, 128), (unsigned)W), dim3(256), 0, r.st,
-                               ws.iter, ws.flagsFT, ws.flagsTF, ws.dataFT, T, Fa, N, N, N, N);
+                               ws.iter, ws.flagsFT, ws.flagsTF, ws.dataFT, T, Fa, N, N, N, N, iter_builds_dead(s) ? ws.dead : (uint8_t*)nullptr);
             break;
         case Begin::Cached:
             rc = launch_u8<0>(r, ws.iter, ws.flagsTF, N, N, N, W);
@@ -1706,7 +1720,7 @@
     if (!rc) rc = launch_colst(r, r.pl.swF, ws.sres, ws.smed, ws.sout, ws.d_chunk_ends, Fa, Wn, (int)r.pl.G, 0, 0, 1);
     if (rc) return rc;
     if (s.spec_or != SpecOr::Scalar)
-        hipLaunchKernelGGL(k_spec_rows, dim3((unsigned)cdiv(nS, 256)), dim3(256), 0, r.st, ws.sout, ws.srows, Fa, Wn);
+        hipLaunchKernelGGL(k_spec_rows, dim3((unsigned)cdiv(nS, 256)), dim3(256), 0, r.st, ws.sout, ws.srows, Fa, Wn, iter_builds_dead(s) ? ws.dead : (uint8_t*)nullptr);
     switch (s.spec_or) {
         case SpecOr::Scalar:
             hipLaunchKernelGGL(k_or_spec, grid1(N, W), dim3(256), 0, r.st, ws.flagsTF, ws.sout, T, Fa, Wn);
@@ -1730,7 +1744,7 @@
     const Ws& ws = r.ws;
     const int T = (int)r.pl.T, Fa = (int)r.pl.Fa;
     bool wrote_panel = false;
-    const int rc = background2d(r, s.ft_current(), s.fused_resid ? ws.residP : nullptr, &wrote_panel);
+    const int rc = background2d(r, s.ft_current(), s.fused_resid ? ws.residP : nullptr, &wrote_panel, iter_builds_dead(s));
     *residTF = wrote_panel ? ws.residP : ws.Aw;
     if (rc || wrote_panel) return rc;
     return launch_transpose<float>(r, ws.Bw, ws.Aw, Fa, T, (size_t)r.pl.PF * T, (size_t)T * Fa, r.Wb, 0.0f, s.panel);
@@ -2287,7 +2301,7 @@
         hipLaunchKernelGGL(k_mr_predict, dim3((unsigned)G, W), dim3(256), 0, st, resid, flags_in, d_ends, rej, T / 4, G, N, N, sc, wsS, ccap, ucap, 0);
         for (unsigned round = 1; round <= 2; round++) {
             hipLaunchKernelGGL(k_mr_pass, dim3((unsigned)cdiv(T / 4, 64), (unsigned)ytiles, W), dim3(256), 0, st, resid, flags_in, flags_out, flags_t4,
-                               d_ends, Fa, T / 4, G, N, N, sc, wsS, ccap, ucap, round);
+                               d_ends, Fa, T / 4, G, N, N, sc, wsS, ccap, ucap, round, (const uint8_t*)nullptr);
             hipLaunchKernelGGL(k_mr_finish, dim3((unsigned)G, W), dim3(256), 0, st, resid, flags_in, flags_out, flags_t4, med, d_ends, rej, Fa, T / 4, G,
                                N, N, sc, wsS, ccap, ucap, round);
         }
```

Result: slower. 3044 Mvis/s (-1.8%).
